# darioShar/DLPM

Measured on AMD Instinct MI355X. Metric: samples/sec at T=1000 (CIFAR-10 32x32, alpha=1.7), higher is better.
Workload: dtype f32 (1x1 / stride-2 convolutions: fp32 operands split exactly into 3 bf16 planes, bf16 MFMA products, fp32 accumulate)

## Files before the change

dlpm_amd/_lib.py:

```python
import ctypes as C
import os

_HERE = os.path.dirname(os.path.abspath(__file__))
LIB_PATH = os.environ.get('DLPM_LIB') or os.path.join(_HERE, 'lib', 'libdlpm_amd.so')

vp, i32, i64, u32, u64, f32, f64 = C.c_void_p, C.c_int32, C.c_int64, C.c_uint32, C.c_uint64, C.c_float, C.c_double

ABI_VERSION = 6
UPD_DLIM, UPD_CLIP, UPD_ADVANCE, SMP_NO_FUSED_MLP, UPD_ELEMENTWISE, SMP_LIM = 1, 2, 4, 8, 16, 32
MEAN_TYPES = {'EPSILON': 0, 'START_X': 1, 'Z': 2, 'PREVIOUS_X': 3}
PRED_TO_XSTART, PRED_CLIP, PRED_TO_EPS, PRED_ELEMENTWISE = 1, 2, 4, 16
LOSS_RESCALE_T, LOSS_ELEMENTWISE = 1, 16
AT_T_Q_SAMPLE, AT_T_PREDICT_EPS, AT_T_PREDICT_XSTART = 0, 1, 2
CONV_AUTO, CONV_F4, CONV_F2, CONV_IGEMM = 0, 1, 2, 3
GEMM_AUTO, GEMM_F32, GEMM_BF16X3 = 0, 1, 2


class MT19937(C.Structure):
    _fields_ = [('key', u32 * 624), ('pos', i32), ('has_cached', i32), ('cached', f64)]


class UpdateArgs(C.Structure):
    _fields_ = [('x_dev', vp), ('eps_dev', vp), ('z_dev', vp), ('t_dev', vp), ('g_dev', vp), ('bg_dev', vp),
                ('bs_dev', vp), ('c_eps_dev', vp), ('c_noise_dev', vp), ('A_dev', vp), ('B', i64), ('D', i64),
# ... 37 lines not shown
                ('conv1_w', vp), ('conv1_b', vp), ('ss', vp), ('ss_stride', i64), ('gn2_w', vp), ('gn2_b', vp), ('conv2_w', vp),
                ('conv2_b', vp), ('skip_w', vp), ('skip_b', vp), ('out', vp), ('stats_out', vp)]


class AttnBlockArgs(C.Structure):
    _fields_ = [('x', vp), ('C', i32), ('heads', i32), ('B', i32), ('H', i32), ('W', i32), ('gn_w', vp), ('gn_b', vp),
                ('qkv_w', vp), ('qkv_b', vp), ('proj_w', vp), ('proj_b', vp), ('out', vp), ('stats_out', vp)]


class SamplerConfig(C.Structure):
    _fields_ = [('unet', vp), ('mlp', vp), ('B', i64), ('C', i32), ('H', i32), ('W', i32), ('T', i32), ('alpha', f64),
                ('clamp_a', f64), ('clamp_eps', f64), ('flags', i32), ('dlim_eta', f32), ('seed', u64),
                ('sample_offset', i64), ('use_graph', i32), ('g', vp), ('bg', vp), ('s', vp), ('bs', vp),
                ('lim_ts', vp), ('lim_tmp', vp), ('lim_cx', vp), ('lim_cs', vp), ('lim_cn', vp), ('in_scale', vp),
                ('mean_type', i32)]


SIGNATURES = {
    'dlpm_last_error': (C.c_char_p, []),
    'dlpm_abi_version': (C.c_int, []),
    'dlpm_prof_enable': (C.c_int, [C.c_int]),
    'dlpm_prof_report': (C.c_int, [C.c_char_p, i64]),
    'dlpm_schedule_f32': (C.c_int, [C.c_int, f64, vp, vp, vp, vp]),
    'dlpm_schedule_exploding_f32': (C.c_int, [C.c_int, f64, vp, vp, vp, vp]),
    'dlpm_mt19937_seed': (C.c_int, [C.POINTER(MT19937), u32]),
    'dlpm_skewed_levy_host_f32': (C.c_int, [C.POINTER(MT19937), f64, i64, f64, vp]),
    'dlpm_randn_host_f32': (C.c_int, [C.POINTER(MT19937), i64, vp]),
    'dlpm_skewed_levy_philox_f32': (C.c_int, [vp, C.c_int, i64, f64, f64, u64, i64, vp]),
    'dlpm_skewed_levy_elem_philox_f32': (C.c_int, [vp, C.c_int, i64, i64, f64, f64, u64, i64, vp]),
    'dlpm_init_state_elem_philox_f32': (C.c_int, [vp, i64, i64, f64, f64, f32, u64, i64, vp]),
    'dlpm_init_state_philox_f32': (C.c_int, [vp, i64, i64, f64, f64, f32, u64, i64, vp]),
    'dlpm_coeff_tables_f32': (C.c_int, [vp, vp, vp, vp, C.c_int, i64, vp, vp, vp, vp]),
    'dlpm_update_f32': (C.c_int, [C.POINTER(UpdateArgs), vp]),
    'dlpm_predict_f32': (C.c_int, [C.POINTER(PredictArgs), vp]),
    'dlpm_fill_scaled_t_f32': (C.c_int, [vp, vp, i32, i64, vp]),
    'dlpm_postprocess_f32': (C.c_int, [vp, vp, i64, f32, C.c_int, vp]),
    'dlpm_scale_by_table_f32': (C.c_int, [vp, vp, i64, vp, vp, vp]),
    'dlpm_lim_tables_f32': (C.c_int, [f64, i32, i32, vp, vp, vp, vp, vp]),
    'dlpm_lim_update_f32': (C.c_int, [C.POINTER(LimUpdateArgs), vp]),
    'dlpm_fill_table_t_f32': (C.c_int, [vp, vp, vp, i32, i64, vp]),
    'dlpm_loss_elements_f32': (C.c_int, [C.POINTER(LossArgs), vp]),
    'dlpm_loss_terms_f32': (C.c_int, [vp, vp, vp, i64, i32, i64, i32, i64, i64, vp]),
    'dlpm_loss_reduce_f32': (C.c_int, [vp, i64, i32, i32, i32, vp, vp, vp, vp]),
    'dlpm_at_t_f32': (C.c_int, [i32, vp, vp, vp, vp, vp, vp, i64, i64, i32, vp]),
    'dlpm_mmd_workspace_bytes': (i64, [i64, i64, i64]),
    'dlpm_mmd_f32': (C.c_int, [vp, i64, vp, i64, i64, f64, i32, f64, vp, i64, vp, vp]),
    'dlpm_images_to_rgb8': (C.c_int, [vp, vp, i64, i32, i32, i32, vp]),
    'dlpm_png_bound': (i64, [i32, i32]),
    'dlpm_png_encode_rgb8': (C.c_int, [vp, i32, i32, i32, vp, i64, C.POINTER(i64)]),
    'dlpm_png_write_rgb8': (C.c_int, [vp, i64, i32, i32, C.c_char_p, i64, i32, i32]),
    'dlpm_unet_create': (C.c_int, [C.POINTER(UNetConfig), C.POINTER(vp)]),
    'dlpm_unet_create_conditional': (C.c_int, [C.POINTER(UNetConfig), i32, C.POINTER(vp)]),
    'dlpm_unet_num_classes': (i32, [vp]),
    'dlpm_unet_set_param': (C.c_int, [vp, C.c_char_p, vp, i64]),
    'dlpm_unet_num_params': (C.c_int, [vp]),
    'dlpm_unet_param_key': (C.c_char_p, [vp, C.c_int, C.POINTER(i64)]),
    'dlpm_unet_finalize': (C.c_int, [vp]),
    'dlpm_unet_workspace_bytes': (i64, [vp, i64]),
    'dlpm_unet_forward': (C.c_int, [vp, vp, vp, vp, i64, vp, i64, vp]),
    'dlpm_unet_forward_uniform_t': (C.c_int, [vp, vp, vp, vp, i64, vp, i64, vp]),
    'dlpm_unet_forward_labels': (C.c_int, [vp, vp, vp, vp, vp, i64, vp, i64, vp]),
    'dlpm_unet_forward_uniform_t_labels': (C.c_int, [vp, vp, vp, vp, vp, i64, vp, i64, vp]),
    'dlpm_unet_forward_update': (C.c_int, [vp, vp, vp, C.POINTER(UpdateArgs), vp, i64, vp, i64, vp]),
    'dlpm_unet_time_embedding_width': (i64, [vp]),
    'dlpm_unet_time_embeddings_scratch_bytes': (i64, [vp, i64]),
    'dlpm_unet_time_embeddings': (C.c_int, [vp, vp, i64, vp, vp, i64, vp]),
    'dlpm_unet_bind_time_table': (C.c_int, [vp, vp, vp]),
    'dlpm_unet_keep_features': (C.c_int, [vp, C.c_int]),
    'dlpm_unet_num_features': (C.c_int, [vp]),
    'dlpm_unet_feature_shape': (C.c_int, [vp, C.c_int, C.POINTER(i32), C.POINTER(i32), C.POINTER(i32)]),
    'dlpm_unet_get_feature': (C.c_int, [vp, C.c_int, vp, i64, vp]),
    'dlpm_unet_flops_per_sample': (i64, [vp]),
    'dlpm_unet_set_conv_policy': (C.c_int, [vp, i32, i64]),
    'dlpm_unet_set_gemm_policy': (C.c_int, [vp, i32]),
    'dlpm_unet_plan_version': (i64, [vp]),
    'dlpm_unet_destroy': (None, [vp]),
    'dlpm_mlp_create': (C.c_int, [i32, i32, i32, i32, C.POINTER(vp)]),
    'dlpm_mlp_set_param': (C.c_int, [vp, C.c_char_p, vp, i64]),
    'dlpm_mlp_finalize': (C.c_int, [vp]),
    'dlpm_mlp_forward': (C.c_int, [vp, vp, vp, vp, i64, vp]),
    'dlpm_mlp_sample_steps_f32': (C.c_int, [vp, vp, vp, vp, vp, i32, i64, i32, i32, u64, i64, vp, vp]),
    'dlpm_mlp_destroy': (None, [vp]),
    'dlpm_conv2d_f32': (C.c_int, [C.POINTER(ConvArgs), vp, vp]),
    'dlpm_groupnorm_coeffs_f32': (C.c_int, [vp, vp, i32, i32, i32, i32, i32, vp, vp, vp, i64, i64, vp, vp, vp]),
    'dlpm_attention_f32': (C.c_int, [vp, vp, i32, i32, i32, i32, vp]),
    'dlpm_attention_general_f32': (C.c_int, [vp, vp, i32, i32, i32, i32, vp]),
    'dlpm_resblock_small_f32': (C.c_int, [C.POINTER(ResBlockArgs), vp, i64, vp]),
    'dlpm_resblock_img_f32': (C.c_int, [C.POINTER(ResBlockArgs), vp, i64, vp]),
    'dlpm_resblock_img_scratch_floats': (i64, [i64, i32]),
    'dlpm_attnblock_small_f32': (C.c_int, [C.POINTER(AttnBlockArgs), vp, i64, vp]),
    'dlpm_timestep_embedding_f32': (C.c_int, [vp, vp, i64, i32, vp]),
    'dlpm_nchw_to_nhwc_f32': (C.c_int, [vp, vp, i32, i32, i32, i32, vp]),
    'dlpm_nhwc_to_nchw_f32': (C.c_int, [vp, vp, i32, i32, i32, i32, vp]),
    'dlpm_sampler_create': (C.c_int, [C.POINTER(SamplerConfig), C.POINTER(vp)]),
    'dlpm_sampler_reseed': (C.c_int, [vp, u64, i64]),
    'dlpm_sampler_begin': (C.c_int, [vp, vp]),
    'dlpm_sampler_begin_injected': (C.c_int, [vp, vp, vp, vp]),
    'dlpm_sampler_set_state': (C.c_int, [vp, vp, i32, vp]),
    'dlpm_sampler_step_injected': (C.c_int, [vp, vp, vp]),
    'dlpm_sampler_steps': (C.c_int, [vp, i32, vp]),
    'dlpm_sampler_set_history': (C.c_int, [vp, vp, vp]),
    'dlpm_sampler_set_labels': (C.c_int, [vp, vp, vp]),
    'dlpm_sampler_copy_state': (C.c_int, [vp, vp, vp]),
    'dlpm_sampler_state': (vp, [vp]),
    'dlpm_sampler_t': (i32, [vp]),
    'dlpm_sampler_table': (vp, [vp, C.c_int]),
    'dlpm_sampler_destroy': (None, [vp]),
}

_lib = None


class DlpmError(RuntimeError):
    pass


def lib():
    global _lib
    if _lib is None:
        if not os.path.exists(LIB_PATH):
            raise DlpmError('libdlpm_amd.so is missing at %s -- run `python -m dlpm_amd.build` '
                            '(or __graft_entry__.build()); there is no CPU fallback' % LIB_PATH)
        handle = C.CDLL(LIB_PATH)
        for name, (res, args) in SIGNATURES.items():
            fn = getattr(handle, name)
            fn.restype = res
            fn.argtypes = args
        got = handle.dlpm_abi_version()
        if got != ABI_VERSION:
            raise DlpmError('libdlpm_amd.so has ABI version %d, the Python mirror expects %d -- rebuild with '
                            '`python -m dlpm_amd.build`' % (got, ABI_VERSION))
        _lib = handle
    return _lib


def check(rc):
    if rc != 0:
        msg = lib().dlpm_last_error().decode('utf-8', 'replace')
        if rc == -1:
            raise ValueError(msg)
        raise DlpmError('[dlpm status %d] %s' % (rc, msg))


def stream_ptr():
    import torch
    return torch.cuda.current_stream().cuda_stream


def ptr(t):
    if t is None:
        return None
    import torch
    assert t.is_contiguous(), 'non-contiguous tensor crossing the C ABI'
    assert t.dtype in (torch.float32, torch.int32), t.dtype
    return t.data_ptr()
```

dlpm_amd/csrc/conv.h:

```cpp
#pragma once
#include "common.h"

namespace dlpm {

struct ConvLaunch {
    const float *src0 = nullptr, *src1 = nullptr;
    int C0 = 0, C1 = 0;
    int B = 0, Hin = 0, Win = 0, Hout = 0, Wout = 0;
    int ks = 1, stride = 1, ups = 0;
    const float *w = nullptr;
    const float *w_frag = nullptr;
    const float *w_wino = nullptr;
    const float *w_wino4 = nullptr;
    const float *w_wino4_n64 = nullptr, *w_wino4_n32 = nullptr;
    const void *w_split = nullptr;
    const float *w_small = nullptr;
    const float *w_taps = nullptr;
    const float *w_hfused = nullptr;
    const float *bias = nullptr;
    const float *coefA = nullptr, *coefB = nullptr;
    int act_silu = 0;
    const float *res0 = nullptr, *res1 = nullptr;
    int R0 = 0;
    float *out = nullptr;
    int Cout = 0;
    int in_nchw = 0, out_nchw = 0;
    int gen = 0;
    int64_t dispatch_B = 0;
    int gemm = 0;
    int ksplit = 0;
    float2 *stats_out = nullptr;
#ifdef DLPM_PHASE_TIMING
    unsigned long long *phase = nullptr;
#endif
};

bool igemm_supported(const ConvLaunch &c);
int launch_conv_igemm(const ConvLaunch &c, hipStream_t st);
int launch_conv_direct(const ConvLaunch &c, hipStream_t st);
int launch_conv_stem(const ConvLaunch &c, hipStream_t st);
struct HeadUpdate {
    float *x = nullptr;
    const float *z = nullptr;
    const int32_t *t = nullptr;
    const float *g = nullptr, *c_eps = nullptr, *c_noise = nullptr;
    const uint64_t *key = nullptr;
    uint64_t seed = 0;
    int64_t sample_offset = 0;
    float *const *hist_pp = nullptr;
    float *eps_out = nullptr;
    int32_t T = 0;
    int64_t B = 0;
};
bool head_conv_ok(const ConvLaunch &c);
int launch_conv_head(const ConvLaunch &c, const HeadUpdate *hu, hipStream_t st);
int relayout_weight_head(const float *oihw_dev, float *dst_dev, int Cout, int Cin, hipStream_t st);
bool head_gemm_ok(const ConvLaunch &c);
int head_taps_rows(int Cout);
int64_t head_gemm_scratch_floats(const ConvLaunch &c);
int launch_conv_head_gemm(const ConvLaunch &c, const HeadUpdate *hu, float *P, hipStream_t st);
int relayout_weight_head_taps(const float *oihw_dev, float *dst_dev, int Cout, int Cin, hipStream_t st);
bool head_fused_ok(const ConvLaunch &c);
int64_t head_fused_weight_floats(int Cin);
int relayout_weight_head_fused(const float *oihw_dev, float *dst_dev, int Cout, int Cin, hipStream_t st);
int launch_conv_head_fused(const ConvLaunch &c, const HeadUpdate *hu, hipStream_t st);
bool wino_geometry(const ConvLaunch &c, int *bh, int *bw, int *nimg);
int wino_tiles(const ConvLaunch &c);
int launch_conv_wino(const ConvLaunch &c, hipStream_t st);
int64_t wino_weight_floats(int Cout, int Cin);
int relayout_weight_wino(const float *oihw_dev, float *dst_dev, int Cout, int Cin, hipStream_t st);
bool wino4_enabled();
bool wino4_geometry(const ConvLaunch &c, int *bh, int *bw, int *nimg);
bool wino4_preferred(const ConvLaunch &c, int *bh, int *bw, int *nimg);
int launch_conv_wino4(const ConvLaunch &c, hipStream_t st);
int64_t wino4_weight_floats(int Cout, int Cin);
int relayout_weight_wino4(const float *oihw_dev, float *dst_dev, int Cout, int Cin, hipStream_t st, int nq = 0);
struct ResImgLaunch {
    const float *x0 = nullptr, *x1 = nullptr;
    int C0 = 0, C1 = 0, B = 0;
    int H = 32;
    const float2 *st0 = nullptr, *st1 = nullptr;
    int nt0 = 1, nt1 = 1;
    const float *coefA1 = nullptr, *coefB1 = nullptr;
    const float *gn1_w = nullptr, *gn1_b = nullptr, *gn2_w = nullptr, *gn2_b = nullptr;
    const float *w1 = nullptr, *b1 = nullptr;
    const float *w2 = nullptr, *b2 = nullptr;
    const float *emb = nullptr;
    int64_t emb_stride = 0;
    int emb_off = 0;
    const float *res = nullptr;
    float *hbuf = nullptr;
    float *out = nullptr;
    float2 *stats_out = nullptr;
#ifdef DLPM_PHASE_TIMING
    unsigned long long *phase = nullptr;
#endif
};
bool res_img_ok(const ResImgLaunch &r);
int launch_resblock_img(const ResImgLaunch &r, hipStream_t st);

bool conv_split_ok(const ConvLaunch &c);
int launch_conv_split(const ConvLaunch &c, hipStream_t st);
int64_t split_weight_floats(int Cout, int Cin, int taps);
int relayout_weight_split(const float *oihw_dev, void *dst_dev, int Cout, int Cin, int taps, hipStream_t st);
int conv_stats_pixels(const ConvLaunch &c);
int conv_ksplit_for(const ConvLaunch &c);
int wino4_launch_nq(const ConvLaunch &c);
int64_t wino_grid_at(const ConvLaunch &c, int64_t B);
int launch_splitk_reduce(const float *part, int S, int64_t npix, int Cout, const float *bias, const float *res0, const float *res1, int R0,
                         float *out, hipStream_t st);
inline int launch_conv_fallback(const ConvLaunch &L, hipStream_t st) {
    if (L.in_nchw && !L.out_nchw && L.ks == 3 && L.stride == 1 && !L.ups && L.C1 == 0 && L.Cout % 4 == 0 && !L.coefA &&
        !L.act_silu && !L.res0 && L.bias)
        return launch_conv_stem(L, st);
    return launch_conv_direct(L, st);
}

int relayout_weight(const float *oihw_dev, float *dst_dev, int Cout, int Cin, int ks, bool for_igemm, hipStream_t st);
int64_t frag_weight_floats(int Cout, int Cin);
int relayout_weight_frag(const float *oihw_dev, float *dst_dev, int Cout, int Cin, hipStream_t st);

int launch_gn_coeffs(const float *src0, const float *src1, int C0, int C1, int B, int HW, int groups,
                     const float *gamma, const float *beta, const float *ss, int64_t ss_stride, int64_t ss_offset,
                     float *coefA, float *coefB, hipStream_t st);
int launch_gn_coeffs_from_stats(const float2 *st0, const float2 *st1, int C0, int C1, int B, int nt0, int nt1, int HW, int groups,
                                const float *gamma, const float *beta, const float *ss, int64_t ss_stride,
                                int64_t ss_offset, float *coefA, float *coefB, hipStream_t st);
int launch_attention(const float *qkv, float *out, int B, int T, int C, int heads, hipStream_t st);
int launch_attention_general(const float *qkv, float *out, int B, int T, int C, int heads, hipStream_t st);

struct ResSmallLaunch {
    const float *x0 = nullptr, *x1 = nullptr;
    int C0 = 0, C1 = 0, B = 0, H = 0, W = 0;
    const float *gn1_w = nullptr, *gn1_b = nullptr, *gn2_w = nullptr, *gn2_b = nullptr;
    const float *w1f = nullptr, *b1 = nullptr;
    const float *w2f = nullptr, *b2 = nullptr;
    const float *wsf = nullptr, *bs = nullptr;
    const float *emb = nullptr;
    int64_t emb_stride = 0;
    int emb_off = 0;
    float *out = nullptr;
    float2 *stats_out = nullptr;
};
struct AttnSmallLaunch {
    const float *x = nullptr;
    int C = 0, heads = 0, B = 0, H = 0, W = 0;
    const float *gn_w = nullptr, *gn_b = nullptr;
    const float *wqkv = nullptr, *bqkv = nullptr;
    const float *wproj = nullptr, *bproj = nullptr;
    float *out = nullptr;
    float2 *stats_out = nullptr;
#ifdef DLPM_PHASE_TIMING
    unsigned long long *phase = nullptr;
#endif
};
bool attn_small_ok(const AttnSmallLaunch &a);
int launch_attnblock_small(const AttnSmallLaunch &a, hipStream_t st);
bool attn16_ok(const AttnSmallLaunch &a);
int launch_attnblock16(const AttnSmallLaunch &a, hipStream_t st);
// ... 18 lines not shown
```

dlpm_amd/csrc/conv_igemm.hip:

```cpp
#include <cstdlib>

#include <algorithm>

#include "conv.h"
#include "igemm_epilogue.h"

namespace dlpm {
namespace {

constexpr int KC = 32;
constexpr int LDS_LD = 36;

template <int BN, int WAVES_M, int WAVES_N, int RM, int RN>
__device__ __forceinline__ void epilogue_rows(const ConvLaunch &p, floatx16 (&acc)[RM][RN], float *lds, int64_t m0, int n0,
                                              int64_t M, int tid, int wm, int wn, int l31, int kh) {
    constexpr int LD = BN + 4, PR = RM * 32, C4 = BN / 4, RG = 256 / C4;
    const int R1 = p.Cout - p.R0;
    const bool do_stats = p.stats_out != nullptr;
    float4 K = make_float4(0.f, 0.f, 0.f, 0.f), s1 = K, s2 = K;
    int cnt = 0;
    for (int ph = 0; ph < WAVES_M; ph++) {
        if (wm == ph) {
#pragma unroll
            for (int i = 0; i < RM; i++)
// ... 913 lines not shown
    return *nimg * (*th + 2) * (W + 2) * 8 <= HALO_NIT * 256;
}

template <int BN, int WAVES_M, int WAVES_N, int RM, int RN, int RING, bool UPS>
static int launch_halo_ws_r(const ConvLaunch &c, int th, int nimg, int64_t grid, hipStream_t st) {
    const int hp = nimg * ((UPS ? th / 2 : th) + 2) * ((UPS ? c.Wout / 2 : c.Wout) + 2);
    size_t shmem = (size_t)((hp + 3) & ~3) * LDS_LD * sizeof(float) + (size_t)nimg * 64 * sizeof(float);
    const size_t epi = (size_t)(RM * 32) * (BN + 4) * sizeof(float);
    const size_t stats = (size_t)(256 / (BN / 4)) * BN * 2 * sizeof(float);
    if (shmem < epi) shmem = epi;
    if (shmem < stats) shmem = stats;
    {
        int r = ensure_dynamic_lds(reinterpret_cast<const void *>(&k_conv3x3_halo_ws<BN, WAVES_M, WAVES_N, RM, RN, RING, UPS>), 64 * 1024);
        if (r != DLPM_OK) return r;
    }
    k_conv3x3_halo_ws<BN, WAVES_M, WAVES_N, RM, RN, RING, UPS><<<(unsigned)grid, 256, shmem, st>>>(c, th, nimg);
    return DLPM_OK;
}

template <int BN, int WAVES_M, int WAVES_N, int RM, int RN>
static int launch_halo_ws(const ConvLaunch &c, int th, int nimg, int64_t grid, hipStream_t st) {
    if (c.ups) return launch_halo_ws_r<BN, WAVES_M, WAVES_N, RM, RN, 2, true>(c, th, nimg, grid, st);
    return launch_halo_ws_r<BN, WAVES_M, WAVES_N, RM, RN, 2, false>(c, th, nimg, grid, st);
}

template <int BN, int WAVES_M, int WAVES_N, int RM, int RN>
static int launch_halo(const ConvLaunch &c, int th, int nimg, int64_t grid, hipStream_t st) {
    const int hp = nimg * (th + 2) * (c.Wout + 2);
    const size_t shmem = (size_t)(((hp + 3) & ~3) + 2 * BN) * LDS_LD * sizeof(float) + (size_t)nimg * 64 * sizeof(float);
    {
        int r = ensure_dynamic_lds(reinterpret_cast<const void *>(&k_conv3x3_halo<BN, WAVES_M, WAVES_N, RM, RN>), 100 * 1024);
        if (r != DLPM_OK) return r;
    }
    k_conv3x3_halo<BN, WAVES_M, WAVES_N, RM, RN><<<(unsigned)grid, 256, shmem, st>>>(c, th, nimg);
    return DLPM_OK;
}

static bool stem_stats_ok(const ConvLaunch &c) {
    const int Cq = c.Cout / 4;
    return c.in_nchw && !c.out_nchw && c.ks == 3 && c.stride == 1 && !c.ups && c.C1 == 0 && (c.C0 == 3 || c.C0 == 1) && c.Cout % 4 == 0 &&
           Cq >= 1 && Cq <= 256 && (Cq & (Cq - 1)) == 0 && ((int64_t)c.Hout * c.Wout) % 1024 == 0;
}

int launch_conv_stem(const ConvLaunch &c, hipStream_t st) {
    const int64_t total = (int64_t)c.B * c.Hout * c.Wout * (c.Cout / 4);
    ProfScope ps("conv_stem", 2.0 * total * 4 * c.C0 * 9, 4.0 * ((double)c.B * c.Hin * c.Win * c.C0 + total * 4.0), st);
    const int Cq = c.Cout / 4;
    const bool regw = Cq >= 1 && Cq <= 256 && (Cq & (Cq - 1)) == 0;
    const int64_t Mpix = (int64_t)c.B * c.Hout * c.Wout;
    const int ppb = 1024;
    if (c.stats_out && !stem_stats_ok(c)) {
        set_error("launch_conv_stem: statistics requested for a shape that cannot emit them");
        return DLPM_ERR_UNSUPPORTED;
    }
    static int nolds = -1;
    if (nolds < 0) { const char *e = getenv("DLPM_NO_STEM_LDS"); nolds = (e && e[0] == '1') ? 1 : 0; }
    const int W = c.Wout;
    const bool lds_ok = !nolds && regw && c.Hin == c.Hout && c.Win == c.Wout && (W & (W - 1)) == 0 && W >= 4 && W <= 64 && ppb % W == 0 &&
                        ((int64_t)c.Hout * W) % ppb == 0 && c.bias;
    if (lds_ok && (c.C0 == 3 || c.C0 == 1)) {
        const size_t shmem = std::max((size_t)(ppb / W + 2) * (W + 2) * sizeof(float4), (size_t)(256 / Cq) * c.Cout * sizeof(float2));
        if (c.C0 == 3) k_conv_stem_lds<3><<<(unsigned)(Mpix / ppb), 256, shmem, st>>>(c, ppb);
        else k_conv_stem_lds<1><<<(unsigned)(Mpix / ppb), 256, shmem, st>>>(c, ppb);
        DLPM_LAUNCH_CHECK();
        return DLPM_OK;
    }
    if (c.C0 == 3 && regw) k_conv_stem_regw<3><<<(unsigned)ceil_div(Mpix, ppb), 256, 0, st>>>(c, ppb);
    else if (c.C0 == 1 && regw) k_conv_stem_regw<1><<<(unsigned)ceil_div(Mpix, ppb), 256, 0, st>>>(c, ppb);
    else if (c.C0 == 3) k_conv_stem<3><<<(unsigned)ceil_div(total, 256), 256, 0, st>>>(c);
    else if (c.C0 == 1) k_conv_stem<1><<<(unsigned)ceil_div(total, 256), 256, 0, st>>>(c);
    else return launch_conv_direct(c, st);
    DLPM_LAUNCH_CHECK();
    return DLPM_OK;
}

int conv_stats_pixels(const ConvLaunch &c) {
    int a, b, n;
    if (conv_ksplit_for(c) > 1) return 0;
    if (c.in_nchw) return stem_stats_ok(c) ? 1024 : 0;
    if (conv_split_ok(c)) {
        const int64_t hw = (int64_t)c.Hout * c.Wout;
        return (c.R0 & 3) ? 0 : hw % BM == 0 ? BM : hw == 64 ? 64 : 0;
    }
    if (wino4_preferred(c, &a, &b, &n)) return n == 1 ? 256 : (n == 4 && a * b == 4) ? 64 : 0;
    if (wino_geometry(c, &a, &b, &n)) return n == 1 ? 4 * wino_tiles(c) : 0;
    if (c.out_nchw || (c.Cout & 3) || (c.R0 & 3)) return 0;
    return ((int64_t)c.Hout * c.Wout) % BM == 0 ? BM : 0;
}

int launch_conv_igemm(const ConvLaunch &c, hipStream_t st) {
    const int64_t M = (int64_t)c.B * c.Hout * c.Wout;
    const int64_t mt = ceil_div(M, BM);
    const double K = (double)(c.C0 + c.C1) * c.ks * c.ks;
    const double bytes = 4.0 * ((double)c.B * c.Hin * c.Win * (c.C0 + c.C1) + K * c.Cout + (double)M * c.Cout * (c.res0 ? 2 : 1));
    char pname[96];
    int th = 0, nimg = 1;
    if (prof_enabled() && prof_detail())
        snprintf(pname, sizeof(pname), "conv%dx%d_igemm:H%d:Cin%d+%d:Cout%d:s%d:u%d:coef%d", c.ks, c.ks, c.Hout, c.C0, c.C1, c.Cout,
                 c.stride, c.ups, c.coefA ? 1 : 0);
    else
        snprintf(pname, sizeof(pname), "%s", c.ks == 3 ? (halo_ok(c, &th, &nimg) ? "conv3x3_halo" : "conv3x3_igemm") : "conv1x1_igemm");
    if (conv_split_ok(c)) {
        if (prof_enabled() && prof_detail())
            snprintf(pname, sizeof(pname), "conv%dx%d_bf16x3:H%d:Cin%d+%d:Cout%d:s%d:coef%d", c.ks, c.ks, c.Hout, c.C0, c.C1, c.Cout, c.stride,
                     c.coefA ? 1 : 0);
        else
            snprintf(pname, sizeof(pname), c.ks == 1 ? "conv1x1_bf16x3" : "conv3x3_bf16x3");
        ProfScope pss(pname, 2.0 * M * c.Cout * K, bytes + 2.0 * K * c.Cout, st);
#ifdef DLPM_PHASE_TIMING
        const_cast<ConvLaunch &>(c).phase = phase_buffer();
#endif
        return launch_conv_split(c, st);
    }
    {
        int wb, ww, wi;
        if (wino4_preferred(c, &wb, &ww, &wi)) {
            if (prof_enabled() && prof_detail())
                snprintf(pname, sizeof(pname), "conv3x3_wino4:H%d:Cin%d+%d:Cout%d:u%d:coef%d", c.Hout, c.C0, c.C1, c.Cout, c.ups, c.coefA ? 1 : 0);
            else
                snprintf(pname, sizeof(pname), "conv3x3_wino4");
            ProfScope psw(pname, 2.0 * M * c.Cout * K, bytes, st);
            return launch_conv_wino4(c, st);
        }
        if (wino_geometry(c, &wb, &ww, &wi)) {
            if (prof_enabled() && prof_detail())
                snprintf(pname, sizeof(pname), "conv3x3_wino:H%d:Cin%d+%d:Cout%d:u%d:coef%d", c.Hout, c.C0, c.C1, c.Cout, c.ups, c.coefA ? 1 : 0);
            else
                snprintf(pname, sizeof(pname), "conv3x3_wino");
            ProfScope psw(pname, 2.0 * M * c.Cout * K, bytes, st);
            return launch_conv_wino(c, st);
        }
    }
    ProfScope ps(pname, 2.0 * M * c.Cout * K, bytes, st);
#ifdef DLPM_PHASE_TIMING
    const_cast<ConvLaunch &>(c).phase = phase_buffer();
#endif
    if (halo_ok(c, &th, &nimg)) {
        int r;
        if (c.w_frag && !ws_disabled() && (c.C0 + c.C1) % KC == 0) {
            if (c.Cout > 64) r = launch_halo_ws<128, 2, 2, 2, 2>(c, th, nimg, mt * ceil_div(c.Cout, 128), st);
            else if (c.Cout > 32) r = launch_halo_ws<64, 2, 2, 2, 1>(c, th, nimg, mt * ceil_div(c.Cout, 64), st);
            else r = launch_halo_ws<32, 4, 1, 1, 1>(c, th, nimg, mt * ceil_div(c.Cout, 32), st);
            if (r != DLPM_OK) return r;
            DLPM_LAUNCH_CHECK();
            return DLPM_OK;
        }
        if (c.Cout > 64) r = launch_halo<128, 2, 2, 2, 2>(c, th, nimg, mt * ceil_div(c.Cout, 128), st);
        else if (c.Cout > 32) r = launch_halo<64, 2, 2, 2, 1>(c, th, nimg, mt * ceil_div(c.Cout, 64), st);
        else r = launch_halo<32, 4, 1, 1, 1>(c, th, nimg, mt * ceil_div(c.Cout, 32), st);
        if (r != DLPM_OK) return r;
        DLPM_LAUNCH_CHECK();
        return DLPM_OK;
    }
    static int nofast = -1;
    if (nofast < 0) { const char *e = getenv("DLPM_NO_FAST_IGEMM"); nofast = (e && e[0] == '1') ? 1 : 0; }
    const int bn = c.Cout > 64 ? 128 : c.Cout > 32 ? 64 : 32;
    const bool full = !nofast && M % BM == 0 && c.Cout % bn == 0 && !c.out_nchw && (c.R0 & 3) == 0;
    const bool g1 = full && c.ks == 1 && c.stride == 1 && !c.ups && !c.in_nchw && c.C0 % KC == 0 && (c.C0 + c.C1) % KC == 0;
    const int mode = g1 ? 2 : full ? 1 : 0;
    const unsigned grid = (unsigned)(mt * ceil_div(c.Cout, bn));
#define DLPM_IGEMM_LAUNCH(BN_, WM_, WN_, RM_, RN_)                                                   \
    do {                                                                                             \
        if (mode == 2) k_conv_igemm<BN_, WM_, WN_, RM_, RN_, 2><<<grid, 256, 0, st>>>(c);            \
        else if (mode == 1) k_conv_igemm<BN_, WM_, WN_, RM_, RN_, 1><<<grid, 256, 0, st>>>(c);       \
        else k_conv_igemm<BN_, WM_, WN_, RM_, RN_, 0><<<grid, 256, 0, st>>>(c);                      \
    } while (0)
    if (bn == 128) DLPM_IGEMM_LAUNCH(128, 2, 2, 2, 2);
    else if (bn == 64) DLPM_IGEMM_LAUNCH(64, 2, 2, 2, 1);
    else DLPM_IGEMM_LAUNCH(32, 4, 1, 1, 1);
#undef DLPM_IGEMM_LAUNCH
    DLPM_LAUNCH_CHECK();
    return DLPM_OK;
}

int64_t frag_weight_floats(int Cout, int Cin) {
    return ((int64_t)((Cout + 31) / 32) * (Cin / 32) * 9 * 4 + 2) * 256;
}

int relayout_weight_frag(const float *oihw_dev, float *dst_dev, int Cout, int Cin, hipStream_t st) {
    const int64_t n = (int64_t)((Cout + 31) / 32) * (Cin / 32) * 9 * 4 * 256;
    DLPM_HIP(hipMemsetAsync(dst_dev + n, 0, 2 * 256 * sizeof(float), st));
    k_relayout_weight_frag<<<(unsigned)ceil_div(n, 256), 256, 0, st>>>(oihw_dev, dst_dev, Cout, Cin);
    DLPM_LAUNCH_CHECK();
    return DLPM_OK;
}

int relayout_weight(const float *oihw_dev, float *dst_dev, int Cout, int Cin, int ks, bool for_igemm, hipStream_t st) {
    const int64_t n = (int64_t)Cout * Cin * ks * ks;
    k_relayout_weight<<<(unsigned)ceil_div(n, 256), 256, 0, st>>>(oihw_dev, dst_dev, Cout, Cin, ks, for_igemm ? 1 : 0);
    DLPM_LAUNCH_CHECK();
    return DLPM_OK;
}

}
```

dlpm_amd/csrc/conv_wino4.hip:

```cpp
#include <cstdlib>
#include <type_traits>

#include "conv.h"
#include "gn_stats.h"

namespace dlpm {
namespace {

typedef float floatx4 __attribute__((ext_vector_type(4)));

constexpr int F4_TILES = 16;
constexpr int F4_NQ = 128;
constexpr int F4_KC = 8;
constexpr int F4_RAWPIX = 576;
constexpr int F4_PRLD = F4_KC + 4;
constexpr int F4_NT = 512;
constexpr int F4_QNIT = (F4_RAWPIX * 2 + F4_NT - 1) / F4_NT;
constexpr int F4_RAWBUF = F4_RAWPIX * F4_PRLD + 16;
constexpr int F4_RAWPIX_N = 400;
constexpr int F4_RAWBUF_N = F4_RAWPIX_N * F4_PRLD + 16;
constexpr int f4_nq_of(int cout) { return cout % 128 == 0 ? 128 : cout % 64 == 0 ? 64 : 32; }
constexpr int F4_CFS = 16 * 2 * F4_KC;
constexpr int F4_VBUF = 36 * F4_TILES * F4_KC;
#ifndef F4_RING_DEPTH
// ... 100 lines not shown
        f4_v_row_out(Ta, vb + 0 * 3 * vpp, vpp);
    } else {
#pragma unroll
        for (int c = 0; c < 6; c++) f4_bt_mid<3>(d, c, Ta[c], Tb[c]);
        f4_v_row_out(Ta, vb + 3 * 3 * vpp, vpp);
        f4_v_row_out(Tb, vb + 4 * 3 * vpp, vpp);
#pragma unroll
        for (int c = 0; c < 6; c++) Tb[c] = f4_bt_outer<5>(d, c);
        f4_v_row_out(Tb, vb + 5 * 3 * vpp, vpp);
    }
}

__device__ __forceinline__ void f4_at(float m0, float m1, float m2, float m3, float m4, float m5, float &y0, float &y1, float &y2, float &y3) {
    const float s12 = m1 + m2, d12 = m1 - m2, s34 = m3 + m4, d34 = m3 - m4;
    y0 = m0 + s12 + s34;
    y1 = fmaf(PB, d34, PA * d12);
    y2 = fmaf(PB2, s34, PA2 * s12);
    y3 = fmaf(PB3, d34, PA3 * d12) + m5;
}
__device__ __forceinline__ void f4_out_tile(const floatx4 (&acc)[36], int r, float (&Yt)[16]) {
    float Z[4][6];
#pragma unroll
    for (int b = 0; b < 6; b++)
        f4_at(acc[0 * 6 + b][r], acc[1 * 6 + b][r], acc[2 * 6 + b][r], acc[3 * 6 + b][r], acc[4 * 6 + b][r], acc[5 * 6 + b][r], Z[0][b], Z[1][b],
              Z[2][b], Z[3][b]);
#pragma unroll
    for (int i = 0; i < 4; i++) f4_at(Z[i][0], Z[i][1], Z[i][2], Z[i][3], Z[i][4], Z[i][5], Yt[i * 4 + 0], Yt[i * 4 + 1], Yt[i * 4 + 2], Yt[i * 4 + 3]);
}

template <int N>
__device__ __forceinline__ void f4_stats_lane(float K, float s1, float s2, float &mean, float &M2) {
    mean = K + s1 * (1.f / N);
    M2 = fmaxf(s2 - s1 * s1 * (1.f / N), 0.f);
}
template <int N>
__device__ __forceinline__ void f4_stats_merge(float K, float s1, float s2, int lane, float &mean, float &M2) {
    f4_stats_lane<N>(K, s1, s2, mean, M2);
    float na = (float)N;
#pragma unroll
    for (int sft = 16; sft <= 32; sft <<= 1) {
        const float om = __shfl_xor(mean, sft), oM2 = __shfl_xor(M2, sft);
        const float lo_m = (lane & sft) ? om : mean, hi_m = (lane & sft) ? mean : om;
        const float lo_M = (lane & sft) ? oM2 : M2, hi_M = (lane & sft) ? M2 : oM2;
        const float dd = hi_m - lo_m;
        mean = lo_m + dd * 0.5f;
        M2 = lo_M + hi_M + dd * dd * (na * 0.5f);
        na *= 2.f;
    }
}

__device__ __forceinline__ void f4_mfma4(float4 aa, float4 b, floatx4 &acc0, floatx4 &acc1) {
    acc0 = __builtin_amdgcn_mfma_f32_16x16x4f32(aa.x, b.x, acc0, 0, 0, 0);
    acc1 = __builtin_amdgcn_mfma_f32_16x16x4f32(aa.z, b.z, acc1, 0, 0, 0);
    acc0 = __builtin_amdgcn_mfma_f32_16x16x4f32(aa.y, b.y, acc0, 0, 0, 0);
    acc1 = __builtin_amdgcn_mfma_f32_16x16x4f32(aa.w, b.w, acc1, 0, 0, 0);
}
__device__ __forceinline__ void f4_mfma_pair(int pp, const float *asrc, int vpp, const float4 *wp, int lane, float4 (&aq)[2], float4 (&bq)[F4_RING],
                                             floatx4 (&acc)[36]) {
    constexpr int AHEAD = F4_RING - 1;
    if (pp == 0) aq[0] = *reinterpret_cast<const float4 *>(asrc);
    if (pp + AHEAD < 18) bq[(pp + AHEAD) % F4_RING] = wp[(pp + AHEAD) * 64 + lane];
    if (pp + 1 < 18) aq[(pp + 1) & 1] = *reinterpret_cast<const float4 *>(asrc + (pp + 1) * vpp);
    f4_mfma4(aq[pp & 1], bq[pp % F4_RING], acc[2 * pp], acc[2 * pp + 1]);
}

__device__ __forceinline__ float4 f4_affine4(float4 x, float4 ca, float4 cb) {
    return make_float4(fmaf(x.x, ca.x, cb.x), fmaf(x.y, ca.y, cb.y), fmaf(x.z, ca.z, cb.z), fmaf(x.w, ca.w, cb.w));
}
__device__ __forceinline__ float4 f4_silu4(float4 x) { return make_float4(silu_f(x.x), silu_f(x.y), silu_f(x.z), silu_f(x.w)); }
__device__ __forceinline__ float4 f4_affine_silu4(float4 x, float4 ca, float4 cb) { return f4_silu4(f4_affine4(x, ca, cb)); }
template <int W, int PRLD>
__device__ __forceinline__ int f4_item_pack(int pix, int ch) {
    constexpr int RW = W + 2;
    const int ry = pix / RW, rx = pix - ry * RW;
    const int iy = ry - 1, ix = rx - 1;
    const bool pad = iy < 0 || iy >= W || ix < 0 || ix >= W;
    const int lo = pix * PRLD + ch + 4 * (ry >> 2);
    return pix >= RW * RW ? (1 << 25) : (lo | (pad ? (1 << 24) : ((iy * W + ix) << 14)));
}
__device__ __forceinline__ int f4_item_lds(int iv) { return iv & 16383; }
__device__ __forceinline__ int f4_item_src(int iv) { return (iv >> 14) & 1023; }
__device__ __forceinline__ bool f4_item_pad(int iv) { return iv & (1 << 24); }
__device__ __forceinline__ bool f4_item_none(int iv) { return iv & (1 << 25); }

template <bool UPS, int QN = F4_QNIT, int NW = 8>
__global__ void __launch_bounds__((NW + (NW == 8 ? 0 : NW == 4 ? 3 : 2)) * 64, NW == 2 ? 2 : 1) k_conv3x3_wino4(ConvLaunch p_in, int bh_in, int bw_in, int nimg_in) {
    constexpr bool HELP = NW != 8;
    constexpr int NH = NW == 8 ? 0 : NW == 4 ? 3 : 2;
    constexpr int F4_NT = (NW + NH) * 64, F4_NQ = NW * 16;
    constexpr int F4_RAWBUF = NW == 8 ? dlpm::F4_RAWBUF : F4_RAWBUF_N;
    ConvLaunch p = p_in;
    const int bh = bh_in, bw = bw_in, nimg = nimg_in;
    extern __shared__ __attribute__((aligned(16))) float wsm[];
    float *V = wsm;
    float *raw = wsm + 2 * F4_VBUF;
    float *Cf = raw + 2 * F4_RAWBUF;

    DLPM_PHASE_DECL;
#ifdef DLPM_PHASE_TIMING
    const long long _c0 = clock64(), _r0 = wall_clock64();
#endif
#ifdef DLPM_PHASE_TIMING
    long long _wait = 0;
#endif
    const int tid = threadIdx.x, lane = tid & 63, wave = tid >> 6;
    const bool mfma_wave = !HELP || wave < NW;
    const int li = lane & 15, lk = lane >> 4;
    const int W = p.Wout, H = p.Hout, TW = W >> 2, TH = H >> 2;
    const int Ws = UPS ? (W >> 1) : W, Hs = UPS ? (H >> 1) : H;
    const int Cin = p.C0 + p.C1;
    int nch = Cin / F4_KC, kb = 0;
    unsigned bid = blockIdx.x, nblk = gridDim.x;
    if constexpr (HELP) {
        if (p.ksplit > 1) {
            nblk = gridDim.x / p.ksplit;
            const int ks = (int)(blockIdx.x / nblk);
            bid = blockIdx.x - (unsigned)ks * nblk;
            nch /= p.ksplit;
            kb = ks * nch;
            p.out += (int64_t)ks * p.B * H * W * p.Cout;
        }
    }
    const int ntn = p.Cout / F4_NQ;
    const int nmb = nblk / ntn;
    const int mb = bid % nmb, n0 = (bid / nmb) * F4_NQ;
    int img0, ty0, tx0, blk_in_img = 0;
    if (nimg == 1) {
        const int bpr = TW / bw, bpi = (TH / bh) * bpr;
        img0 = mb / bpi;
        blk_in_img = mb - img0 * bpi;
        ty0 = (blk_in_img / bpr) * bh;
        tx0 = (blk_in_img % bpr) * bw;
    } else {
        img0 = mb * nimg;
        ty0 = tx0 = 0;
    }
    const int RH = UPS ? 2 * bh + 2 : 4 * bh + 2, RW = UPS ? 2 * bw + 2 : 4 * bw + 2;
    const int oy = UPS ? 2 * ty0 - 1 : 4 * ty0 - 1, ox = UPS ? 2 * tx0 - 1 : 4 * tx0 - 1;
    const int rpi = RH * RW, npix = nimg * rpi;

    const int squad = tid & 1;
    auto pix_of = [&](int it) { return it == 1 ? (F4_NT / 2) + ((F4_NT - 1 - tid) >> 1) : it * (F4_NT / 2) + (tid >> 1); };
    const bool skewed = !UPS && nimg == 1 && bh <= 4;
    int off[QN], lo[QN];
#pragma unroll
    for (int it = 0; it < QN; it++) {
        const int pix = pix_of(it);
        const int img = min(pix / rpi, nimg - 1), r = pix - img * rpi;
        const int ry = r / RW, rx = r - ry * RW;
        const int iy = oy + ry, ix = ox + rx;
        const bool pad = iy < 0 || iy >= Hs || ix < 0 || ix >= Ws || (img0 + img) >= p.B;
        off[it] = pix >= npix ? -2 : (pad ? -1 : (((img0 + img) * Hs + iy) * Ws + ix));
        lo[it] = (pix * F4_PRLD + squad * 4 + (skewed ? 4 * (ry >> 2) : 0)) | ((img * 2 * F4_KC + squad * 4) << 16);
    }
    const bool has_coef = p.coefA != nullptr;
    const int cf_img = tid >> 2, cf_isb = (tid >> 1) & 1;
    const bool cf_mine = has_coef && tid < nimg * 4;
    const float *cf_base = has_coef ? ((cf_isb ? p.coefB : p.coefA) + (int64_t)min(img0 + cf_img, p.B - 1) * Cin + kb * F4_KC + squad * 4) : nullptr;
    float4 xr[QN], cfr = make_float4(0.f, 0.f, 0.f, 0.f);
    auto load_raw_into = [&](float4 (&dst)[QN], int chunk) {
        const int c = (kb + chunk) * F4_KC + squad * 4;
        const bool first = c < p.C0;
        const float *sb = first ? p.src0 + c : p.src1 + (c - p.C0);
        const int ld = first ? p.C0 : p.C1;
#pragma unroll
        for (int it = 0; it < QN; it++) dst[it] = *reinterpret_cast<const float4 *>(sb + (int64_t)max(off[it], 0) * ld);
// ... 134 lines not shown
    if (p.phase && lane == 0) atomicAdd(p.phase + 16 + wave, (unsigned long long)_wait);
#endif

    const int64_t pix0 = ((int64_t)img0 * H + 4 * ty0) * W + 4 * tx0;
    const int ch = n0 + 16 * wave + li;
    const float bias_v = p.bias ? p.bias[ch] : 0.f;
    const bool has_res = p.res0 != nullptr;
    const bool res_first = __builtin_amdgcn_readfirstlane(n0 + 16 * wave) < p.R0;
    const float *res_u = has_res ? (res_first ? p.res0 : p.res1 - p.R0) : nullptr;
    const int res_ld = res_first ? p.R0 : p.Cout - p.R0;
    const int lbw = 31 - __builtin_clz(bw), lbhw = 31 - __builtin_clz(bh * bw);
    float *__restrict__ out_blk = p.out + pix0 * p.Cout;
    const float *__restrict__ res_blk = has_res ? res_u + pix0 * res_ld : nullptr;
    const bool img_stats = p.stats_out != nullptr && nimg == 4 && bh * bw == 4;
    const bool do_stats = (p.stats_out != nullptr && nimg == 1) || img_stats;
    float K = 0.f, s1 = 0.f, s2 = 0.f;
    float rs_all[HELP ? 4 : 1][16] = {};
#pragma unroll
    for (int r = 0; r < 4; r++) {
        const int tile = 4 * lk + r;
        const int timg = tile >> lbhw, ty = (tile & (bh * bw - 1)) >> lbw, tx = tile & (bw - 1);
        const int tpix = (timg * H + 4 * ty) * W + 4 * tx;
        const bool ok = img0 + timg < p.B;
        float rs[16];
        const uint32_t bo_o = (uint32_t)(tpix * p.Cout + ch) * 4u, bo_r = (uint32_t)(tpix * res_ld + ch) * 4u;
        if (HELP) {
            if (r == 0 && has_res) {
#pragma unroll
                for (int rr = 0; rr < 4; rr++) {
                    const int t2 = 4 * lk + rr;
                    const int tp2 = ((t2 >> lbhw) * H + 4 * ((t2 & (bh * bw - 1)) >> lbw)) * W + 4 * (t2 & (bw - 1));
                    const uint32_t b2 = (uint32_t)(tp2 * res_ld + ch) * 4u;
                    const bool ok2 = img0 + (t2 >> lbhw) < p.B;
#pragma unroll
                    for (int k = 0; k < 16; k++)
                        rs_all[rr][k] = ok2 ? *reinterpret_cast<const float *>(reinterpret_cast<const char *>(res_blk + ((k >> 2) * W + (k & 3)) * res_ld) + b2) : 0.f;
                }
            }
#pragma unroll
            for (int k = 0; k < 16; k++) rs[k] = rs_all[r][k];
        } else if (has_res && ok) {
#pragma unroll
            for (int i = 0; i < 4; i++)
#pragma unroll
                for (int j = 0; j < 4; j++)
                    rs[i * 4 + j] = *reinterpret_cast<const float *>(reinterpret_cast<const char *>(res_blk + (i * W + j) * res_ld) + bo_r);
        }
        float Yt[16];
        f4_out_tile(acc, r, Yt);
        if (!ok) continue;
#pragma unroll
        for (int i = 0; i < 4; i++) {
            const float *y = Yt + 4 * i;
#pragma unroll
            for (int j = 0; j < 4; j++) {
                float v = y[j] + bias_v;
                if (has_res) v += rs[i * 4 + j];
                if (do_stats) {
                    if (r == 0 && i == 0 && j == 0) K = v;
                    const float dd = v - K;
                    s1 += dd;
                    s2 = fmaf(dd, dd, s2);
                }
                *reinterpret_cast<float *>(reinterpret_cast<char *>(out_blk + (i * W + j) * p.Cout) + bo_o) = v;
            }
        }
    }
    if (img_stats) {
        if (img0 + lk < p.B) {
            float mean, M2;
            f4_stats_lane<64>(K, s1, s2, mean, M2);
            p.stats_out[(int64_t)(img0 + lk) * p.Cout + ch] = make_float2(mean, M2);
        }
    } else if (do_stats) {
        float mean, M2;
        f4_stats_merge<64>(K, s1, s2, lane, mean, M2);
        if (lk == 0) p.stats_out[((int64_t)img0 * ((H * W) / 256) + blk_in_img) * p.Cout + ch] = make_float2(mean, M2);
    }
    DLPM_PHASE(p, 10);
    DLPM_PHASE_FLUSH(p, 8);
#ifdef DLPM_PHASE_DEFER
    if (p.phase && lane == 0) atomicAdd(p.phase + 16 + wave, (unsigned long long)_wait);
#endif
#ifdef DLPM_PHASE_TIMING
    if (p.phase && tid == 0) {
        atomicAdd(p.phase + 11, 1ull);
        atomicAdd(p.phase + 12, (unsigned long long)(clock64() - _c0));
        atomicAdd(p.phase + 13, (unsigned long long)(wall_clock64() - _r0));
    }
#endif
}

constexpr int FI_TILES = 64, FI_RW = 34, FI_NPIX = FI_RW * FI_RW, FI_NT = 512;
constexpr int FI_QN = (FI_NPIX * 2 + FI_NT - 1) / FI_NT;
constexpr int FI_RAWBUF = FI_NPIX * F4_PRLD + 48;
constexpr int FI_VPP = 4 * FI_TILES * 4;
constexpr int FI_VBUF = 18 * FI_VPP;

#define F4_LDS_BARRIER()                                                  \
    do {                                                                  \
        __builtin_amdgcn_fence(__ATOMIC_RELEASE, "workgroup", "local");   \
        __builtin_amdgcn_s_barrier();                                     \
        __builtin_amdgcn_fence(__ATOMIC_ACQUIRE, "workgroup", "local");   \
    } while (0)

__global__ void __launch_bounds__(FI_NT, 1) k_conv3x3_wino4_img(ConvLaunch p) {
    extern __shared__ __attribute__((aligned(16))) float wsm[];
    float *V = wsm;
    float *raw = V + FI_VBUF;
    float *Cf = raw + FI_RAWBUF;
    DLPM_PHASE_DECL;
#ifdef DLPM_PHASE_TIMING
    const long long _c0 = clock64(), _r0 = wall_clock64();
#endif
    constexpr int H = 32, W = 32;
    const int tid = threadIdx.x, lane = tid & 63, wave = __builtin_amdgcn_readfirstlane(tid >> 6);
    const int li = lane & 15, lk = lane >> 4;
    const int mb = wave >> 1, nw = wave & 1;
    const int img = blockIdx.x;
    const int Cin = p.C0 + p.C1, nch = Cin / F4_KC, last = nch - 1;
    const bool has_coef = p.coefA != nullptr;

    const int squad = tid & 1;
    int itm[FI_QN];
#pragma unroll
    for (int it = 0; it < FI_QN; it++) itm[it] = f4_item_pack<W, F4_PRLD>(it * (FI_NT / 2) + (tid >> 1), squad * 4);
    float4 xr[FI_QN];
    auto load_raw = [&](int chunk) {
        const int c = chunk * F4_KC + squad * 4;
        const bool first = c < p.C0;
        const int ld = first ? p.C0 : p.C1;
        const float *sb = (first ? p.src0 + c : p.src1 + (c - p.C0)) + (int64_t)img * (H * W) * ld;
#pragma unroll
        for (int it = 0; it < FI_QN; it++) xr[it] = *reinterpret_cast<const float4 *>(sb + f4_item_src(itm[it]) * ld);
    };
    auto store_raw = [&](int chunk) {
        const int c = chunk * F4_KC + squad * 4;
        float4 ca = make_float4(1.f, 1.f, 1.f, 1.f), cb = make_float4(0.f, 0.f, 0.f, 0.f);
        if (has_coef) {
            ca = *reinterpret_cast<const float4 *>(Cf + c);
            cb = *reinterpret_cast<const float4 *>(Cf + Cin + c);
        }
#pragma unroll
        for (int it = 0; it < FI_QN; it++) {
            int iv = itm[it];
            asm volatile("" : "+v"(iv));
            if (f4_item_none(iv)) continue;
            float4 x = xr[it];
            if (has_coef) x = f4_affine4(x, ca, cb);
            if (p.act_silu) x = f4_silu4(x);
            if (f4_item_pad(iv)) x = make_float4(0.f, 0.f, 0.f, 0.f);
            *reinterpret_cast<float4 *>(raw + f4_item_lds(iv)) = x;
        }
    };

    int rbase, vofs;
    {
        const int tg = wave & 3, tile = lane & 15, pair = lane >> 4;
        const int ty = 4 * (tg >> 1) + (tile >> 2), tx = 4 * (tg & 1) + (tile & 3);
        rbase = (4 * ty * FI_RW + 4 * tx) * F4_PRLD + pair * 2 + 4 * ty;
        vofs = (pair * FI_TILES + 16 * tg + tile) * 4;
    }
    const int th = wave >> 2;
    auto transform = [&]() { f4_transform_half(th, F4Patch<false, F4_PRLD>{raw + rbase, FI_RW, true}, V + vofs, FI_VPP); };

    const float4 *__restrict__ wp = reinterpret_cast<const float4 *>(p.w_wino4) + (int64_t)nw * nch * 18 * 64;
// ... 485 lines not shown
    auto epilogue = [&](auto ra_c) __attribute__((always_inline)) {
        constexpr int RA = decltype(ra_c)::value;
        exchange(ra_c);
        int chv = ch, lkv = lk;
        asm volatile("" : "+v"(chv), "+v"(lkv));
        const float bias_v = p.b2[chv];
        const int64_t pix0 = (int64_t)img * H * W;
        float *__restrict__ out_blk = p.out + pix0 * CO;
        const float *__restrict__ res_blk = p.res + pix0 * CO;
        const bool do_stats = p.stats_out != nullptr;
        float K = 0.f, s1 = 0.f, s2 = 0.f;
        auto one = [&](auto r_c, int rr) __attribute__((always_inline)) {
            const int tile = 4 * lkv + RA + rr;
            const int tpix = (4 * (tile >> 2)) * W + 4 * (tile & 3);
            float rs[16];
#pragma unroll
            for (int k = 0; k < 16; k++) rs[k] = res_blk[(tpix + (k >> 2) * W + (k & 3)) * CO + chv];
            float Yt[16];
            f4_out_tile(acc, decltype(r_c)::value, Yt);
#pragma unroll
            for (int k = 0; k < 16; k++) {
                const float v = (Yt[k] + bias_v) + rs[k];
                if (rr == 0 && k == 0) K = v;
                const float dd = v - K;
                s1 += dd;
                s2 = fmaf(dd, dd, s2);
                out_blk[(tpix + (k >> 2) * W + (k & 3)) * CO + chv] = v;
            }
        };
        one(std::integral_constant<int, RA>(), 0);
        one(std::integral_constant<int, RA + 1>(), 1);
        if (do_stats) {
            float mean, M2;
            f4_stats_merge<32>(K, s1, s2, lane, mean, M2);
            if (lkv == 0) part[kh * CO + chv] = make_float2(mean, M2);
            F4_LDS_BARRIER();
            if (kh == 0 && lkv == 0) {
                const float2 a = part[chv], b = part[CO + chv];
                const float dd = b.x - a.x;
                p.stats_out[(int64_t)img * CO + chv] = make_float2(a.x + dd * 0.5f, a.y + b.y + dd * dd * 64.f);
            }
        }
    };
    if (kh == 0) epilogue(std::integral_constant<int, 0>());
    else epilogue(std::integral_constant<int, 2>());
    DLPM_PHASE(p, 10);
    DLPM_PHASE_FLUSH(p, 8);
#ifdef DLPM_PHASE_TIMING
    if (p.phase && tid == 0) atomicAdd(p.phase + 11, 1ull);
#endif
}

__global__ void k_relayout_weight_wino4(const float *oihw, float *dst, int Cout, int Cin, int nw) {
    const int nch = Cin / F4_KC;
    const int64_t total = (int64_t)Cout * Cin * 36;
    const int64_t i = (int64_t)blockIdx.x * blockDim.x + threadIdx.x;
    if (i >= total) return;
    const int e = (int)(i & 3);
    const int lane = (int)((i >> 2) & 63);
    int64_t r = i >> 8;
    const int pp = (int)(r % 18); r /= 18;
    const int chunk = (int)(r % nch); r /= nch;
    const int wave = (int)(r % nw);
    const int nt = (int)(r / nw);
    const int lk = lane >> 4, li = lane & 15;
    const int pos = 2 * pp + (e >> 1);
    const int cin = chunk * F4_KC + 2 * lk + (e & 1);
    const int cout = nt * (16 * nw) + wave * 16 + li;
    const float *g = oihw + ((int64_t)cout * Cin + cin) * 9;
    const double a = F4_PA, b = F4_PB, a2 = a * a, b2 = b * b;
    const double n0 = a2 * b2, na = 2. * a2 * (a2 - b2), nb = 2. * b2 * (b2 - a2);
    const double G[6][3] = {{1. / n0, 0., 0.},         {1. / na, a / na, a2 / na}, {1. / na, -a / na, a2 / na},
                            {1. / nb, b / nb, b2 / nb}, {1. / nb, -b / nb, b2 / nb}, {0., 0., 1.}};
    const int ra = pos / 6, rb = pos % 6;
    double u = 0.;
    for (int ii = 0; ii < 3; ii++) {
        double row = 0.;
        for (int jj = 0; jj < 3; jj++) row += (double)g[ii * 3 + jj] * G[rb][jj];
        u += G[ra][ii] * row;
    }
    dst[i] = (float)u;
}

int f4_mode() {
    static int v = -1;
    if (v < 0) { const char *e = getenv("DLPM_WINO_F4"); v = e ? atoi(e) : 1; }
    return v;
}

}

bool wino4_enabled() { return f4_mode() != 0; }

static bool narrow_enabled() {
    static int v = -1;
    if (v < 0) { const char *e = getenv("DLPM_WINO4_NARROW"); v = e ? atoi(e) : 1; }
    return v != 0;
}

static bool wino4_geometry_nq(const ConvLaunch &c, int nq, int *bh, int *bw, int *nimg) {
    if (nq != F4_NQ && !narrow_enabled()) return false;
    if (!c.w_wino4 || c.ks != 3 || c.stride != 1 || c.in_nchw || c.out_nchw) return false;
    if ((c.Hout & 3) || (c.Wout & 3) || c.Cout % 32 != 0 || (c.C0 + c.C1) % F4_KC != 0 || c.C0 % F4_KC != 0) return false;
    const int rawpix = nq == F4_NQ ? F4_RAWPIX : F4_RAWPIX_N;
    if ((c.R0 & 15) != 0) return false;
    const int TH = c.Hout / 4, TW = c.Wout / 4;
    int h, w, n;
    if (TH * TW >= F4_TILES) {
        w = TW < 4 ? TW : 4;
        if (F4_TILES % w != 0) return false;
        h = F4_TILES / w;
        if (TW % w != 0 || TH % h != 0) return false;
        n = 1;
    } else {
        if (F4_TILES % (TH * TW) != 0) return false;
        h = TH; w = TW; n = F4_TILES / (TH * TW);
    }
    const int RH = c.ups ? 2 * h + 2 : 4 * h + 2, RW = c.ups ? 2 * w + 2 : 4 * w + 2;
    if (n * RH * RW > rawpix) return false;
    *bh = h; *bw = w; *nimg = n;
    return true;
}

static int wino4_nq_for(const ConvLaunch &c) {
    const int base = f4_nq_of(c.Cout);
    if (base != F4_NQ || c.dispatch_B <= 0 || (!c.w_wino4_n64 && !c.w_wino4_n32)) return base;
    static int floor_nq = -1;
    if (floor_nq < 0) { const char *e = getenv("DLPM_WINO4_NQ"); floor_nq = e ? atoi(e) : 32; }
    int best = F4_NQ;
    for (int nq = F4_NQ; nq >= 32 && nq >= floor_nq; nq >>= 1) {
        if (nq == 64 && !c.w_wino4_n64) continue;
        if (nq == 32 && !c.w_wino4_n32) continue;
        int h, w, n;
        if (!wino4_geometry_nq(c, nq, &h, &w, &n)) continue;
        best = nq;
        const int64_t tiles = c.dispatch_B * (c.Hout / 4) * (c.Wout / 4);
        const int64_t mblocks = n == 1 ? tiles / F4_TILES : ceil_div(c.dispatch_B, (int64_t)n);
        if (mblocks * (c.Cout / nq) >= 256) break;
    }
    return best;
}

bool wino4_geometry(const ConvLaunch &c, int *bh, int *bw, int *nimg) { return wino4_geometry_nq(c, wino4_nq_for(c), bh, bw, nimg); }
int wino4_launch_nq(const ConvLaunch &c) { return wino4_nq_for(c); }

bool wino4_preferred(const ConvLaunch &c, int *bh, int *bw, int *nimg) {
    if (c.gen == DLPM_CONV_F2 || c.gen == DLPM_CONV_IGEMM) return false;
    if (!wino4_geometry(c, bh, bw, nimg)) return false;
    if (!c.w_wino || c.gen == DLPM_CONV_F4) return true;
    if (*nimg > 4) return false;
    if (c.dispatch_B <= 0) return true;
    const int64_t tiles = c.dispatch_B * (c.Hout / 4) * (c.Wout / 4);
    const int64_t mblocks = *nimg == 1 ? tiles / F4_TILES : ceil_div(c.dispatch_B, (int64_t)*nimg);
    return mblocks * (c.Cout / wino4_nq_for(c)) >= 256;
}

static bool wino4_whole_image(const ConvLaunch &c) {
    static int v = -1;
    if (v < 0) { const char *e = getenv("DLPM_WINO4_IMG"); v = e ? atoi(e) : 1; }
    return v != 0 && c.Cout == 32 && !c.ups && c.Hout == 32 && c.Wout == 32 && (c.C0 + c.C1) <= 1024;
}

static int launch_conv_wino4_nq(const ConvLaunch &c, int nq, int bh, int bw, int nimg, hipStream_t st);

int launch_conv_wino4(const ConvLaunch &c, hipStream_t st) {
    int bh, bw, nimg;
// ... 31 lines not shown
        KFn fn = nq == 64 ? (c.ups ? &k_conv3x3_wino4<true, 2, 4> : &k_conv3x3_wino4<false, 2, 4>)
                          : (c.ups ? &k_conv3x3_wino4<true, 4, 2> : &k_conv3x3_wino4<false, 4, 2>);
        const int r = ensure_dynamic_lds(reinterpret_cast<const void *>(fn), 160 * 1024);
        if (r != DLPM_OK) return r;
        const size_t lds = (size_t)(2 * F4_VBUF + 2 * F4_RAWBUF_N + 2 * F4_CFS) * sizeof(float);
        const int ks = c.ksplit > 1 ? c.ksplit : 1;
        if (ks > 1 && (c.bias || c.res0 || c.stats_out || ((c.C0 + c.C1) / F4_KC) % ks != 0)) {
            set_error("launch_conv_wino4: a split-K launch carries no bias / residual / statistics and divides its chunks evenly");
            return DLPM_ERR_ARG;
        }
        fn<<<(unsigned)(mblocks * (c.Cout / nq) * ks), (nq == 64 ? 7 : 4) * 64, lds, st>>>(c, bh, bw, nimg);
        DLPM_LAUNCH_CHECK();
        return DLPM_OK;
    }
    if (c.ksplit > 1) {
        set_error("launch_conv_wino4: split-K is a narrow-shape launch");
        return DLPM_ERR_ARG;
    }
    const int RHp = c.ups ? 2 * bh + 2 : 4 * bh + 2, RWp = c.ups ? 2 * bw + 2 : 4 * bw + 2;
    const bool small = nimg * RHp * RWp <= F4_NT;
    KFn fn = c.ups ? (small ? &k_conv3x3_wino4<true, 2> : &k_conv3x3_wino4<true>) : (small ? &k_conv3x3_wino4<false, 2> : &k_conv3x3_wino4<false>);
    const int r = ensure_dynamic_lds(reinterpret_cast<const void *>(fn), 160 * 1024);
    if (r != DLPM_OK) return r;
    const size_t lds = (size_t)(2 * F4_VBUF + 2 * F4_RAWBUF + 2 * F4_CFS) * sizeof(float);
    fn<<<(unsigned)(mblocks * (c.Cout / F4_NQ)), F4_NT, lds, st>>>(c, bh, bw, nimg);
    DLPM_LAUNCH_CHECK();
    return DLPM_OK;
}

bool res_img_ok(const ResImgLaunch &r) {
    static int v = -1;
    if (v < 0) { const char *e = getenv("DLPM_RES_IMG"); v = e ? atoi(e) : 1; }
    const int Cin = r.C0 + r.C1;
    const bool common = v != 0 && wino4_enabled() && r.w1 && r.w2 && r.res && Cin <= 128 && Cin >= 32 &&
                        (r.st0 ? (r.C1 == 0 || r.st1 != nullptr) : (r.coefA1 && r.coefB1));
    if (r.H == 16) {
        static int v16 = -1;
        if (v16 < 0) { const char *e = getenv("DLPM_RES_IMG16"); v16 = e ? atoi(e) : 1; }
        return common && v16 != 0 && Cin % F6_KC == 0 && r.C0 % F6_KC == 0;
    }
    return common && r.H == 32 && r.hbuf && Cin % F4_KC == 0 && r.C0 % F4_KC == 0;
}

int launch_resblock_img(const ResImgLaunch &r, hipStream_t st) {
    if (!res_img_ok(r)) {
        set_error("launch_resblock_img: unsupported block");
        return DLPM_ERR_UNSUPPORTED;
    }
    const int Cin = r.C0 + r.C1;
#ifdef DLPM_PHASE_TIMING
    const_cast<ResImgLaunch &>(r).phase = phase_buffer();
#endif
    if (r.H == 16) {
        const double M16 = (double)r.B * 256;
        ProfScope ps16("resblock_img:H16", 2.0 * M16 * 64 * 9.0 * (Cin + 64), 4.0 * (M16 * (Cin + 64 + 64) + 64 * 9.0 * (Cin + 64)), st);
        const int e16 = ensure_dynamic_lds(reinterpret_cast<const void *>(&k_resblock_wino4_img16), 160 * 1024);
        if (e16 != DLPM_OK) return e16;
        const size_t lds16 = (size_t)(F6_VBUF + F6_RAWBUF + F6_HBUF + 256 + 512 + 256 + F6_QN * FI_NT) * sizeof(float);
        k_resblock_wino4_img16<<<(unsigned)r.B, FI_NT, lds16, st>>>(r);
        DLPM_LAUNCH_CHECK();
        return DLPM_OK;
    }
    const double M = (double)r.B * 1024;
    ProfScope ps("resblock_img:H32", 2.0 * M * 32 * 9.0 * (Cin + 32), 4.0 * (M * (Cin + 32 + 32) + 32 * 9.0 * (Cin + 32)), st);
    const int e = ensure_dynamic_lds(reinterpret_cast<const void *>(&k_resblock_wino4_img), 160 * 1024);
    if (e != DLPM_OK) return e;
    const size_t lds = (size_t)(FI_VBUF + FI_RAWBUF + 256 + 512 + 256 + FI_QN * FI_NT) * sizeof(float);
    k_resblock_wino4_img<<<(unsigned)r.B, FI_NT, lds, st>>>(r);
    DLPM_LAUNCH_CHECK();
    return DLPM_OK;
}

int64_t wino4_weight_floats(int Cout, int Cin) { return (int64_t)Cout * Cin * 36 + F4_PAD * 256; }

int relayout_weight_wino4(const float *oihw_dev, float *dst_dev, int Cout, int Cin, hipStream_t st, int nq_in) {
    const int64_t n = (int64_t)Cout * Cin * 36;
    DLPM_HIP(hipMemsetAsync(dst_dev + n, 0, (size_t)F4_PAD * 256 * sizeof(float), st));
    const int nq = nq_in > 0 ? nq_in : f4_nq_of(Cout);
    k_relayout_weight_wino4<<<(unsigned)ceil_div(n, 256), 256, 0, st>>>(oihw_dev, dst_dev, Cout, Cin, nq / 16);
    DLPM_LAUNCH_CHECK();
    return DLPM_OK;
}

}
```

dlpm_amd/csrc/unet.hip:

```cpp
#include <cmath>
#include <cstdlib>
#include <map>
#include <string>
#include <utility>
#include <vector>

#include "conv.h"

using namespace dlpm;

namespace {

struct Param {
    std::string key;
    int64_t numel = 0;
    float *dev = nullptr;
    bool set = false;
};

enum LayerKind { L_STEM, L_RES, L_ATTN, L_DOWN, L_UP };

struct ConvW {
    int p_w = -1, p_b = -1;
    int cout = 0, cin = 0, ks = 1;
    bool use_igemm = false;
    float *w_dev = nullptr;
    float *w_frag = nullptr;
    float *w_wino = nullptr;
    float *w_wino4 = nullptr;
    float *w_wino4_n64 = nullptr, *w_wino4_n32 = nullptr;
    float *w_small = nullptr;
    float *w_taps = nullptr;
    void *w_split = nullptr;
    float *w_rs = nullptr;
    float *w_hfused = nullptr;
    bool owns = false;
};

struct Layer {
    LayerKind kind;
    std::string pre;
    int cin = 0, cout = 0;
    int emb_off = 0;
    ConvW c1, c2, skip;
    bool has_skip = false;
    int p_gn1_w = -1, p_gn1_b = -1, p_gn2_w = -1, p_gn2_b = -1;
    int p_emb_w = -1, p_emb_b = -1;
};

struct Tensor4 {
    float *p = nullptr;
    int C = 0, H = 0, W = 0;
    float2 *stats = nullptr;
    int stats_px = 0;
};

struct Bump {
    char *base = nullptr;
    int64_t cap = 0, off = 0, peak = 0;
    bool dry = false, overflow = false, reuse = true;
    std::vector<std::pair<int64_t, int64_t>> holes;
    std::map<int64_t, int64_t> live;
    char *origin() const { return dry ? reinterpret_cast<char *>(uintptr_t(1) << 20) : base; }
    float *alloc(int64_t nfloats) {
        const int64_t bytes = (nfloats * 4 + 255) / 256 * 256;
        int64_t at = -1;
        if (reuse) {
            size_t best = holes.size();
            for (size_t i = 0; i < holes.size(); i++)
                if (holes[i].second >= bytes && (best == holes.size() || holes[i].second < holes[best].second)) best = i;
            if (best != holes.size()) {
                at = holes[best].first;
                if (holes[best].second == bytes) holes.erase(holes.begin() + best);
                else { holes[best].first += bytes; holes[best].second -= bytes; }
            }
        }
        if (at < 0) {
            at = off;
            off += bytes;
            if (off > peak) peak = off;
            if (!dry && off > cap) overflow = true;
        }
        live[at] = bytes;
        return reinterpret_cast<float *>(origin() + at);
    }
    void release(const void *p) {
        if (!p || !reuse) return;
        const int64_t at = reinterpret_cast<const char *>(p) - origin();
        auto it = live.find(at);
        if (it == live.end()) return;
        int64_t lo = at, n = it->second;
        live.erase(it);
        size_t i = 0;
        while (i < holes.size() && holes[i].first < lo) i++;
        if (i > 0 && holes[i - 1].first + holes[i - 1].second == lo) { lo = holes[i - 1].first; n += holes[i - 1].second; holes.erase(holes.begin() + --i); }
        if (i < holes.size() && lo + n == holes[i].first) { n += holes[i].second; holes.erase(holes.begin() + i); }
        if (lo + n == off) { off = lo; return; }
        holes.insert(holes.begin() + i, std::make_pair(lo, n));
    }
};

void policy_of(const dlpm_unet *u, ConvLaunch &L);

void plan_stats(const dlpm_unet *u, Bump &ws, Tensor4 &t, const ConvW &c, int B, int C0, int stride, int ups, bool stem = false) {
    static int off = -1;
    if (off < 0) { const char *e = getenv("DLPM_NO_GN_FUSION"); off = (e && e[0] == '1') ? 1 : 0; }
    t.stats = nullptr;
    t.stats_px = 0;
    if (off || (!c.use_igemm && !stem)) return;
    ConvLaunch L;
    L.w_wino = c.w_wino; L.w_wino4 = c.w_wino4; L.w_wino4_n64 = c.w_wino4_n64; L.w_wino4_n32 = c.w_wino4_n32; L.w_split = c.w_split; L.ks = c.ks; L.stride = stride; L.ups = ups; L.Hout = t.H; L.Wout = t.W; L.Cout = c.cout;
    L.Hin = ups ? t.H / 2 : t.H * stride; L.Win = ups ? t.W / 2 : t.W * stride;
    L.C0 = C0; L.C1 = c.cin - C0; L.B = B;
    L.in_nchw = stem ? 1 : 0;
    policy_of(u, L);
    const int px = conv_stats_pixels(L);
    if (px <= 0) return;
    t.stats_px = px;
    t.stats = reinterpret_cast<float2 *>(ws.alloc((int64_t)2 * B * (t.H * t.W / px) * t.C));
}

int gn_any(Tensor4 x0, Tensor4 x1, int B, int groups, const float *gamma, const float *beta, const float *ss,
           int64_t ss_stride, int64_t ss_offset, float *cA, float *cB, hipStream_t st) {
    const int HW = x0.H * x0.W;
    if (x0.stats && (x1.C == 0 || x1.stats))
        return launch_gn_coeffs_from_stats(x0.stats, x1.stats, x0.C, x1.C, B, HW / x0.stats_px, x1.C ? HW / x1.stats_px : 1, HW,
                                           groups, gamma, beta, ss, ss_stride, ss_offset, cA, cB, st);
    return launch_gn_coeffs(x0.p, x1.p, x0.C, x1.C, B, HW, groups, gamma, beta, ss, ss_stride, ss_offset, cA, cB, st);
}


void drop(Bump &ws, Tensor4 &t) {
    ws.release(t.p);
    ws.release(t.stats);
    t.p = nullptr;
    t.stats = nullptr;
}

}

struct dlpm_unet {
    dlpm_unet_config cfg;
    std::vector<Param> params;
    std::map<std::string, int> index;
    std::vector<std::vector<Layer>> in_blocks, out_blocks;
    std::vector<Layer> mid;
    std::vector<int> skip_ch;
    ConvW te0, te2, embcat, head;
    int p_head_gn_w = -1, p_head_gn_b = -1;
    float *embcat_w = nullptr, *embcat_b = nullptr;
    int emb_total = 0, ted = 0, final_ch = 0;
    int num_classes = 0;
    int p_label = -1;
    bool finalized = false;
    std::vector<Tensor4> feats;
    int64_t flops = 0;
    bool keep_feats = false;
    int gen = DLPM_CONV_AUTO;
    int64_t dispatch_B = 0;
    int gemm = DLPM_GEMM_AUTO;
    int64_t plan_version = 0;

    int add(const std::string &key, int64_t numel) {
        Param p;
        p.key = key;
        p.numel = numel;
        params.push_back(p);
        index[key] = (int)params.size() - 1;
        return (int)params.size() - 1;
    }
    ConvW conv(const std::string &pre, int cout, int cin, int ks) {
        ConvW c;
        c.cout = cout; c.cin = cin; c.ks = ks;
        c.p_w = add(pre + "weight", (int64_t)cout * cin * ks * ks);
        c.p_b = add(pre + "bias", cout);
        return c;
    }
    Layer res(const std::string &pre, int cin, int cout) {
        Layer L;
        L.kind = L_RES; L.pre = pre; L.cin = cin; L.cout = cout;
        L.p_gn1_w = add(pre + "in_layers.0.weight", cin);
        L.p_gn1_b = add(pre + "in_layers.0.bias", cin);
        L.c1 = conv(pre + "in_layers.2.", cout, cin, 3);
        L.p_emb_w = add(pre + "emb_layers.1.weight", (int64_t)2 * cout * ted);
        L.p_emb_b = add(pre + "emb_layers.1.bias", 2 * cout);
        L.p_gn2_w = add(pre + "out_layers.0.weight", cout);
        L.p_gn2_b = add(pre + "out_layers.0.bias", cout);
        L.c2 = conv(pre + "out_layers.3.", cout, cout, 3);
        L.has_skip = cin != cout;
        if (L.has_skip) L.skip = conv(pre + "skip_connection.", cout, cin, 1);
        L.emb_off = emb_total;
        emb_total += 2 * cout;
        return L;
    }
// ... 9 lines not shown
    bool has_attn(int ds) const {
        for (int i = 0; i < cfg.n_attn; i++)
            if (cfg.attention_resolutions[i] == ds) return true;
        return false;
    }
};

namespace {

void policy_of(const dlpm_unet *u, ConvLaunch &L) {
    L.gen = u->gen;
    L.dispatch_B = u->dispatch_B;
    L.gemm = u->gemm;
}

void build_arch(dlpm_unet *u) {
    const dlpm_unet_config &c = u->cfg;
    const int mc = c.model_channels;
    u->ted = 4 * mc;
    u->te0 = u->conv("time_embed.0.", u->ted, mc, 1);
    u->te2 = u->conv("time_embed.2.", u->ted, u->ted, 1);
    if (u->num_classes > 0) u->p_label = u->add("label_emb.weight", (int64_t)u->num_classes * u->ted);
    {
        Layer L;
        L.kind = L_STEM; L.pre = "input_blocks.0.0."; L.cin = c.in_channels; L.cout = mc;
        L.c1 = u->conv(L.pre, mc, c.in_channels, 3);
        u->in_blocks.push_back({L});
        u->skip_ch.push_back(mc);
    }
    int ch = mc, ds = 1;
    for (int level = 0; level < c.n_mult; level++) {
        const int mult = c.channel_mult[level];
        for (int r = 0; r < c.num_res_blocks; r++) {
            const std::string pre = "input_blocks." + std::to_string(u->in_blocks.size()) + ".";
            std::vector<Layer> seq;
            seq.push_back(u->res(pre + "0.", ch, mult * mc));
            ch = mult * mc;
            if (u->has_attn(ds)) seq.push_back(u->attn(pre + "1.", ch));
            u->in_blocks.push_back(seq);
            u->skip_ch.push_back(ch);
        }
        if (level != c.n_mult - 1) {
            Layer L;
            L.kind = L_DOWN; L.pre = "input_blocks." + std::to_string(u->in_blocks.size()) + ".0.op.";
            L.cin = L.cout = ch;
            L.c1 = u->conv(L.pre, ch, ch, 3);
            u->in_blocks.push_back({L});
            u->skip_ch.push_back(ch);
            ds *= 2;
        }
    }
    u->mid.push_back(u->res("middle_block.0.", ch, ch));
    u->mid.push_back(u->attn("middle_block.1.", ch));
    u->mid.push_back(u->res("middle_block.2.", ch, ch));
    std::vector<int> stack = u->skip_ch;
    for (int level = c.n_mult - 1; level >= 0; level--) {
        const int mult = c.channel_mult[level];
        for (int i = 0; i <= c.num_res_blocks; i++) {
            const std::string pre = "output_blocks." + std::to_string(u->out_blocks.size()) + ".";
            const int ich = stack.back();
            stack.pop_back();
            std::vector<Layer> seq;
            seq.push_back(u->res(pre + "0.", ch + ich, mc * mult));
            ch = mc * mult;
            int k = 1;
            if (u->has_attn(ds)) seq.push_back(u->attn(pre + std::to_string(k++) + ".", ch));
            if (level && i == c.num_res_blocks) {
                Layer L;
                L.kind = L_UP; L.pre = pre + std::to_string(k++) + ".conv.";
                L.cin = L.cout = ch;
                L.c1 = u->conv(L.pre, ch, ch, 3);
                seq.push_back(L);
                ds /= 2;
            }
            u->out_blocks.push_back(seq);
        }
    }
    u->final_ch = ch;
    u->p_head_gn_w = u->add("out.0.weight", ch);
    u->p_head_gn_b = u->add("out.0.bias", ch);
    u->head = u->conv("out.2.", c.out_channels, mc, 3);
}

int prep_conv(dlpm_unet *u, ConvW &c, int C0, int boundary) {
    ConvLaunch probe;
    probe.C0 = C0; probe.C1 = c.cin - C0; probe.Cout = c.cout; probe.ks = c.ks;
    probe.in_nchw = boundary == 1; probe.out_nchw = boundary == 2;
    c.use_igemm = igemm_supported(probe);
    const float *src = u->params[c.p_w].dev;
    if (c.use_igemm && c.ks == 1) {
        c.w_dev = const_cast<float *>(src);
        if (small_weight_ok(c.cout, c.cin, 1) && boundary == 0) {
            DLPM_HIP(hipMalloc(&c.w_rs, (size_t)small_weight_floats(c.cout, c.cin, 1) * sizeof(float)));
            int r = relayout_weight_small(src, c.w_rs, c.cout, c.cin, 1, nullptr);
            if (r != DLPM_OK) return r;
        }
        if (c.cout % 128 == 0 && c.cin % 32 == 0 && boundary == 0) {
            DLPM_HIP(hipMalloc(&c.w_split, (size_t)split_weight_floats(c.cout, c.cin, 1) * sizeof(float)));
            return relayout_weight_split(src, c.w_split, c.cout, c.cin, 1, nullptr);
        }
        return DLPM_OK;
    }
    DLPM_HIP(hipMalloc(&c.w_dev, (size_t)c.cout * c.cin * c.ks * c.ks * sizeof(float)));
    c.owns = true;
    if (c.ks == 3 && c.cout <= 4 && c.cin % 32 == 0) {
        DLPM_HIP(hipMalloc(&c.w_small, (size_t)9 * c.cin * 4 * sizeof(float)));
        int r = relayout_weight_head(src, c.w_small, c.cout, c.cin, nullptr);
        if (r != DLPM_OK) return r;
        if (c.cout <= 3) {
            DLPM_HIP(hipMalloc(&c.w_taps, (size_t)head_taps_rows(c.cout) * c.cin * sizeof(float)));
            r = relayout_weight_head_taps(src, c.w_taps, c.cout, c.cin, nullptr);
            if (r != DLPM_OK) return r;
            if (c.cin <= 128) {
                DLPM_HIP(hipMalloc(&c.w_hfused, (size_t)head_fused_weight_floats(c.cin) * sizeof(float)));
                r = relayout_weight_head_fused(src, c.w_hfused, c.cout, c.cin, nullptr);
                if (r != DLPM_OK) return r;
            }
        }
    }
    if (c.use_igemm && c.ks == 3 && boundary == 4 && c.cout % 128 == 0 && c.cin % 32 == 0) {
        DLPM_HIP(hipMalloc(&c.w_split, (size_t)split_weight_floats(c.cout, c.cin, 9) * sizeof(float)));
        int r = relayout_weight_split(src, c.w_split, c.cout, c.cin, 9, nullptr);
        if (r != DLPM_OK) return r;
    }
    if (c.use_igemm && c.ks == 3 && c.cin % 32 == 0) {
        DLPM_HIP(hipMalloc(&c.w_frag, (size_t)frag_weight_floats(c.cout, c.cin) * sizeof(float)));
        int r = relayout_weight_frag(src, c.w_frag, c.cout, c.cin, nullptr);
        if (r != DLPM_OK) return r;
        if (c.cout % 64 == 0 && c.cin % 16 == 0 && boundary == 0) {
            DLPM_HIP(hipMalloc(&c.w_wino, (size_t)wino_weight_floats(c.cout, c.cin) * sizeof(float)));
            r = relayout_weight_wino(src, c.w_wino, c.cout, c.cin, nullptr);
            if (r != DLPM_OK) return r;
        }
        if (wino4_enabled() && c.cout % 32 == 0 && c.cin % 8 == 0 && boundary == 0) {
            DLPM_HIP(hipMalloc(&c.w_wino4, (size_t)wino4_weight_floats(c.cout, c.cin) * sizeof(float)));
            r = relayout_weight_wino4(src, c.w_wino4, c.cout, c.cin, nullptr);
            if (r != DLPM_OK) return r;
        }
    }
    if (small_weight_ok(c.cout, c.cin, c.ks) && boundary == 0) {
        DLPM_HIP(hipMalloc(&c.w_rs, (size_t)small_weight_floats(c.cout, c.cin, c.ks) * sizeof(float)));
        int r = relayout_weight_small(src, c.w_rs, c.cout, c.cin, c.ks, nullptr);
        if (r != DLPM_OK) return r;
    }
    return relayout_weight(src, c.w_dev, c.cout, c.cin, c.ks, c.use_igemm, nullptr);
}

void attach_conv(const dlpm_unet *u, const ConvW &c, ConvLaunch &L) {
    policy_of(u, L);
    L.w = c.w_dev;
    L.w_frag = c.w_frag;
    L.w_wino = c.w_wino;
    L.w_wino4 = c.w_wino4;
    L.w_wino4_n64 = c.w_wino4_n64;
    L.w_wino4_n32 = c.w_wino4_n32;
    L.w_small = c.w_small;
    L.w_taps = c.w_taps;
    L.w_hfused = c.w_hfused;
    L.w_split = c.w_split;
    L.ks = c.ks;
    L.Cout = c.cout;
}

int run_conv(const dlpm_unet *u, const ConvW &c, ConvLaunch L, hipStream_t st, const HeadUpdate *hu = nullptr, float *head_scratch = nullptr) {
    policy_of(u, L);
    L.w = c.w_dev;
    L.w_frag = c.w_frag;
    L.w_wino = c.w_wino;
    L.w_wino4 = c.w_wino4;
    L.w_wino4_n64 = c.w_wino4_n64;
    L.w_wino4_n32 = c.w_wino4_n32;
    L.w_small = c.w_small;
    L.w_taps = c.w_taps;
    L.w_hfused = c.w_hfused;
    L.w_split = c.w_split;
    L.ks = c.ks;
    L.Cout = c.cout;
    if (head_fused_ok(L)) return launch_conv_head_fused(L, hu, st);
    if (head_scratch && head_gemm_ok(L)) return launch_conv_head_gemm(L, hu, head_scratch, st);
    if (head_conv_ok(L)) return launch_conv_head(L, hu, st);
    if (hu) { set_error("unet: the head convolution of this net cannot carry the fused update"); return DLPM_ERR_UNSUPPORTED; }
    return c.use_igemm ? launch_conv_igemm(L, st) : launch_conv_fallback(L, st);
}

#define TRY(expr)                  \
    do {                           \
        int _r = (expr);           \
        if (_r != DLPM_OK) return _r; \
    } while (0)

struct Ctx {
    dlpm_unet *u;
    int B;
    Bump ws;
    hipStream_t st;
    float *embout = nullptr;
    bool uniform_t = false;
    const int64_t *y = nullptr;
    int64_t emb_pitch() const { return (uniform_t && !y) ? 0 : u->emb_total; }
    const HeadUpdate *hu = nullptr;
    bool dry() const { return ws.dry; }
};

int ksplit_of(const Ctx &cx, const ConvW &c, ConvLaunch L) {
    attach_conv(cx.u, c, L);
    L.bias = nullptr;
    return conv_ksplit_for(L);
}
int run_conv3(Ctx &cx, const ConvW &c, const ConvLaunch &L) {
    const int S = ksplit_of(cx, c, L);
    if (S <= 1) return run_conv(cx.u, c, L, cx.st);
    const int64_t npix = (int64_t)L.B * L.Hout * L.Wout;
    float *part = cx.ws.alloc((int64_t)S * npix * c.cout);
    ConvLaunch P = L;
    P.bias = nullptr; P.res0 = nullptr; P.res1 = nullptr; P.R0 = 0; P.stats_out = nullptr; P.out = part; P.ksplit = S;
    int rc = run_conv(cx.u, c, P, cx.st);
    if (rc == DLPM_OK) rc = launch_splitk_reduce(part, S, npix, c.cout, L.bias, L.res0, L.res1, L.R0, L.out, cx.st);
    cx.ws.release(part);
    return rc;
}
void reserve_ksplit(Ctx &cx, const ConvW &c, const ConvLaunch &L) {
    const int S = ksplit_of(cx, c, L);
    if (S > 1) cx.ws.release(cx.ws.alloc((int64_t)S * L.B * L.Hout * L.Wout * c.cout));
}

void release_res_temps(Ctx &cx, float *cA1, float *cB1, Tensor4 &h1, float *cA2, float *cB2, float *sk) {
    cx.ws.release(cA1);
    cx.ws.release(cB1);
    drop(cx.ws, h1);
    cx.ws.release(cA2);
    cx.ws.release(cB2);
    cx.ws.release(sk);
}

int run_res(Ctx &cx, const Layer &L, Tensor4 x0, Tensor4 x1, Tensor4 *out) {
    dlpm_unet *u = cx.u;
    const int B = cx.B, H = x0.H, W = x0.W, HW = H * W;
    const int C0 = x0.C, C1 = x1.C, Cin = C0 + C1, Co = L.cout;
    {
        ResSmallLaunch r;
        r.x0 = x0.p; r.x1 = x1.p; r.C0 = C0; r.C1 = C1; r.B = B; r.H = H; r.W = W;
        r.w1f = L.c1.w_rs; r.w2f = L.c2.w_rs; r.wsf = L.has_skip ? L.skip.w_rs : nullptr;
        if (u->gen == DLPM_CONV_AUTO && Co == 64 && (!L.has_skip || r.wsf) && res_small_ok(r)) {
            float *o = cx.ws.alloc((int64_t)B * HW * Co);
            out->p = o; out->C = Co; out->H = H; out->W = W;
            out->stats = reinterpret_cast<float2 *>(cx.ws.alloc((int64_t)2 * B * Co));
            out->stats_px = HW;
            if (cx.dry()) return DLPM_OK;
            r.gn1_w = u->params[L.p_gn1_w].dev; r.gn1_b = u->params[L.p_gn1_b].dev;
            r.gn2_w = u->params[L.p_gn2_w].dev; r.gn2_b = u->params[L.p_gn2_b].dev;
            r.b1 = u->params[L.c1.p_b].dev; r.b2 = u->params[L.c2.p_b].dev;
            r.bs = L.has_skip ? u->params[L.skip.p_b].dev : nullptr;
            r.emb = cx.embout; r.emb_stride = cx.emb_pitch(); r.emb_off = L.emb_off;
            r.out = o; r.stats_out = out->stats;
// ... 314 lines not shown
                case L_STEM: convf(L.c1, H, H); break;
                case L_RES:
                    convf(L.c1, H, H); convf(L.c2, H, H);
                    if (L.has_skip) convf(L.skip, H, H);
                    break;
                case L_ATTN:
                    convf(L.c1, H, H); convf(L.c2, H, H);
                    f += 4LL * (H * H) * (H * H) * L.cin;
                    break;
                case L_DOWN: H = (H - 1) / 2 + 1; convf(L.c1, H, H); break;
                case L_UP: H *= 2; convf(L.c1, H, H); break;
            }
        }
    };
    for (auto &s : u->in_blocks) seqf(s);
    seqf(u->mid);
    for (auto &s : u->out_blocks) seqf(s);
    convf(u->head, H, H);
    return f;
}

}

static int create_net(const dlpm_unet_config *cfg, int32_t num_classes, dlpm_unet **out) {
    DLPM_CHECK_ARG(cfg && out, "dlpm_unet_create: null argument");
    DLPM_CHECK_ARG(cfg->in_channels > 0 && cfg->model_channels > 0 && cfg->out_channels > 0 && cfg->num_res_blocks > 0,
                   "dlpm_unet_create: channels / res blocks must be positive");
    DLPM_CHECK_ARG(cfg->n_mult > 0 && cfg->n_mult <= 8 && cfg->n_attn >= 0 && cfg->n_attn <= 8,
                   "dlpm_unet_create: bad channel_mult / attention_resolutions length");
    DLPM_CHECK_ARG(cfg->num_heads > 0 && cfg->image_size > 0, "dlpm_unet_create: bad num_heads / image_size");
    DLPM_CHECK_ARG(cfg->image_size % (1 << (cfg->n_mult - 1)) == 0,
                   "dlpm_unet_create: image_size %d not divisible by 2^%d (the reference UNet fails on such sizes too)",
                   cfg->image_size, cfg->n_mult - 1);
    dlpm_unet *u = new dlpm_unet();
    u->cfg = *cfg;
    u->num_classes = num_classes;
    build_arch(u);
    *out = u;
    return DLPM_OK;
}

extern "C" int dlpm_unet_create(const dlpm_unet_config *cfg, dlpm_unet **out) { return create_net(cfg, 0, out); }

extern "C" int dlpm_unet_create_conditional(const dlpm_unet_config *cfg, int32_t num_classes, dlpm_unet **out) {
    DLPM_CHECK_ARG(num_classes > 0, "dlpm_unet_create_conditional: num_classes must be positive, got %d", num_classes);
    return create_net(cfg, num_classes, out);
}

extern "C" int32_t dlpm_unet_num_classes(const dlpm_unet *net) { return net ? net->num_classes : 0; }

extern "C" int dlpm_unet_num_params(const dlpm_unet *net) { return net ? (int)net->params.size() : 0; }

extern "C" const char *dlpm_unet_param_key(const dlpm_unet *net, int i, int64_t *numel_out) {
    if (!net || i < 0 || i >= (int)net->params.size()) return nullptr;
    if (numel_out) *numel_out = net->params[i].numel;
    return net->params[i].key.c_str();
}

extern "C" int dlpm_unet_set_param(dlpm_unet *net, const char *key, const float *host, int64_t numel) {
    DLPM_CHECK_ARG(net && key && host, "dlpm_unet_set_param: null argument");
    auto it = net->index.find(key);
    DLPM_CHECK_ARG(it != net->index.end(), "dlpm_unet_set_param: unexpected key '%s' for this architecture", key);
    Param &p = net->params[it->second];
    DLPM_CHECK_ARG(p.numel == numel, "dlpm_unet_set_param: '%s' has %lld elements, expected %lld", key, (long long)numel,
                   (long long)p.numel);
    if (!p.dev) DLPM_HIP(hipMalloc(&p.dev, (size_t)numel * sizeof(float)));
    DLPM_HIP(hipMemcpy(p.dev, host, (size_t)numel * sizeof(float), hipMemcpyHostToDevice));
    p.set = true;
    net->finalized = false;
    return DLPM_OK;
}

static void free_conv(ConvW &c) {
    if (c.owns && c.w_dev) (void)hipFree(c.w_dev);
    if (c.w_frag) (void)hipFree(c.w_frag);
    c.w_frag = nullptr;
    if (c.w_wino) (void)hipFree(c.w_wino);
    c.w_wino = nullptr;
    if (c.w_wino4) (void)hipFree(c.w_wino4);
    c.w_wino4 = nullptr;
    if (c.w_wino4_n64) (void)hipFree(c.w_wino4_n64);
    if (c.w_wino4_n32) (void)hipFree(c.w_wino4_n32);
    c.w_wino4_n64 = c.w_wino4_n32 = nullptr;
    if (c.w_small) (void)hipFree(c.w_small);
    c.w_small = nullptr;
    if (c.w_taps) (void)hipFree(c.w_taps);
    c.w_taps = nullptr;
    if (c.w_rs) (void)hipFree(c.w_rs);
    c.w_rs = nullptr;
    if (c.w_hfused) (void)hipFree(c.w_hfused);
    c.w_hfused = nullptr;
    if (c.w_split) (void)hipFree(c.w_split);
    c.w_split = nullptr;
    c.w_dev = nullptr;
    c.owns = false;
}

static void for_each_conv(dlpm_unet *u, void (*fn)(ConvW &)) {
    auto seq = [&](std::vector<Layer> &s) {
        for (auto &L : s) {
            fn(L.c1);
            if (L.kind == L_RES || L.kind == L_ATTN) fn(L.c2);
            if (L.kind == L_RES && L.has_skip) fn(L.skip);
        }
    };
    for (auto &s : u->in_blocks) seq(s);
    seq(u->mid);
    for (auto &s : u->out_blocks) seq(s);
    fn(u->te0);
    fn(u->te2);
    fn(u->head);
}

constexpr int64_t NARROW_COPIES_MAX_BATCH = 512;
static int narrow_wino4_copies(dlpm_unet *u) {
    const bool want = u->dispatch_B > 0 && u->dispatch_B <= NARROW_COPIES_MAX_BATCH;
    int rc = DLPM_OK;
    auto one = [&](ConvW &c) {
        if (rc != DLPM_OK || !c.w_wino4 || c.cout % 128 != 0) return;
        if (!want) {
            if (c.w_wino4_n64) (void)hipFree(c.w_wino4_n64);
            if (c.w_wino4_n32) (void)hipFree(c.w_wino4_n32);
            c.w_wino4_n64 = c.w_wino4_n32 = nullptr;
            return;
        }
        for (int nq : {64, 32}) {
            float *&dst = nq == 64 ? c.w_wino4_n64 : c.w_wino4_n32;
            if (dst) continue;
            if (hipMalloc(&dst, (size_t)wino4_weight_floats(c.cout, c.cin) * sizeof(float)) != hipSuccess) { dst = nullptr; rc = DLPM_ERR_HIP; set_error("narrow_wino4_copies: hipMalloc failed"); return; }
            rc = relayout_weight_wino4(u->params[c.p_w].dev, dst, c.cout, c.cin, nullptr, nq);
            if (rc != DLPM_OK) return;
        }
    };
    auto seq = [&](std::vector<Layer> &s) {
        for (auto &L : s) {
            one(L.c1);
            if (L.kind == L_RES) one(L.c2);
        }
    };
    for (auto &s : u->in_blocks) seq(s);
    seq(u->mid);
    for (auto &s : u->out_blocks) seq(s);
    if (rc == DLPM_OK && hipDeviceSynchronize() != hipSuccess) { set_error("narrow_wino4_copies: synchronize failed"); rc = DLPM_ERR_HIP; }
    return rc;
}

extern "C" int dlpm_unet_finalize(dlpm_unet *u) {
    DLPM_CHECK_ARG(u, "dlpm_unet_finalize: null handle");
    for (auto &p : u->params)
        if (!p.set) {
            set_error("dlpm_unet_finalize: parameter '%s' was never set", p.key.c_str());
            return DLPM_ERR_STATE;
        }
    for_each_conv(u, free_conv);
    auto prep_seq = [&](std::vector<Layer> &s, int C0_first) -> int {
        for (size_t i = 0; i < s.size(); i++) {
            Layer &L = s[i];
            const bool cat = (i == 0 && L.kind == L_RES && C0_first > 0);
            const int C0 = cat ? C0_first : L.c1.cin;
            TRY(prep_conv(u, L.c1, L.kind == L_STEM ? L.c1.cin : C0, L.kind == L_STEM ? 1 : L.kind == L_DOWN ? 4 : 0));
            if (L.kind == L_RES || L.kind == L_ATTN) TRY(prep_conv(u, L.c2, L.c2.cin, 0));
            if (L.kind == L_RES && L.has_skip) TRY(prep_conv(u, L.skip, cat ? C0_first : L.skip.cin, 0));
        }
        return DLPM_OK;
    };
    for (auto &s : u->in_blocks) TRY(prep_seq(s, 0));
    TRY(prep_seq(u->mid, 0));
    {
        int ch = u->mid.back().cout;
        for (auto &s : u->out_blocks) {
            TRY(prep_seq(s, ch));
            ch = s[0].cout;
        }
    }
    TRY(prep_conv(u, u->te0, u->te0.cin, 3));
    TRY(prep_conv(u, u->te2, u->te2.cin, 3));
    TRY(prep_conv(u, u->head, u->head.cin, 2));
    if (u->embcat_w) (void)hipFree(u->embcat_w);
    if (u->embcat_b) (void)hipFree(u->embcat_b);
    DLPM_HIP(hipMalloc(&u->embcat_w, (size_t)u->emb_total * u->ted * sizeof(float)));
    DLPM_HIP(hipMalloc(&u->embcat_b, (size_t)u->emb_total * sizeof(float)));
    auto cat_seq = [&](std::vector<Layer> &s) -> int {
        for (auto &L : s)
            if (L.kind == L_RES) {
                DLPM_HIP(hipMemcpy(u->embcat_w + (size_t)L.emb_off * u->ted, u->params[L.p_emb_w].dev,
                                   (size_t)2 * L.cout * u->ted * sizeof(float), hipMemcpyDeviceToDevice));
                DLPM_HIP(hipMemcpy(u->embcat_b + L.emb_off, u->params[L.p_emb_b].dev, (size_t)2 * L.cout * sizeof(float),
                                   hipMemcpyDeviceToDevice));
            }
        return DLPM_OK;
    };
    for (auto &s : u->in_blocks) TRY(cat_seq(s));
    TRY(cat_seq(u->mid));
    for (auto &s : u->out_blocks) TRY(cat_seq(s));
    u->embcat.cout = u->emb_total; u->embcat.cin = u->ted; u->embcat.ks = 1;
    {
        ConvLaunch probe;
        probe.C0 = u->ted; probe.Cout = u->emb_total; probe.ks = 1;
        u->embcat.use_igemm = igemm_supported(probe);
        if (u->embcat.use_igemm) {
            u->embcat.w_dev = u->embcat_w;
        } else {
            DLPM_HIP(hipMalloc(&u->embcat.w_dev, (size_t)u->emb_total * u->ted * sizeof(float)));
            u->embcat.owns = true;
            TRY(relayout_weight(u->embcat_w, u->embcat.w_dev, u->emb_total, u->ted, 1, false, nullptr));
        }
    }
    TRY(narrow_wino4_copies(u));
    DLPM_HIP(hipDeviceSynchronize());
    u->flops = count_flops(u);
    u->finalized = true;
    u->plan_version++;
    return DLPM_OK;
}

extern "C" int dlpm_unet_set_conv_policy(dlpm_unet *u, int32_t generation, int64_t dispatch_batch) {
    DLPM_CHECK_ARG(u, "dlpm_unet_set_conv_policy: null handle");
    DLPM_CHECK_ARG(generation >= DLPM_CONV_AUTO && generation <= DLPM_CONV_IGEMM, "dlpm_unet_set_conv_policy: unknown generation %d",
                   generation);
    DLPM_CHECK_ARG(dispatch_batch >= 0, "dlpm_unet_set_conv_policy: negative dispatch batch");
    if (u->gen == generation && u->dispatch_B == dispatch_batch) return DLPM_OK;
    u->gen = generation;
    u->dispatch_B = dispatch_batch;
    u->plan_version++;
    if (u->finalized) TRY(narrow_wino4_copies(u));
    return DLPM_OK;
}

extern "C" int dlpm_unet_set_gemm_policy(dlpm_unet *u, int32_t mode) {
    DLPM_CHECK_ARG(u, "dlpm_unet_set_gemm_policy: null handle");
    DLPM_CHECK_ARG(mode >= DLPM_GEMM_AUTO && mode <= DLPM_GEMM_BF16X3, "dlpm_unet_set_gemm_policy: unknown mode %d", mode);
    if (u->gemm == mode) return DLPM_OK;
    u->gemm = mode;
    u->plan_version++;
    return DLPM_OK;
}

extern "C" int64_t dlpm_unet_time_embedding_width(const dlpm_unet *u) { return u ? u->emb_total : -1; }
extern "C" int64_t dlpm_unet_time_embeddings_scratch_bytes(const dlpm_unet *u, int64_t M) {
    return (u && M > 0) ? M * (u->cfg.model_channels + 2 * (int64_t)u->ted) * (int64_t)sizeof(float) : -1;
}

extern "C" int dlpm_unet_time_embeddings(dlpm_unet *net, const float *t_dev, int64_t M, float *out_dev, void *scratch_dev, int64_t scratch_bytes,
// ... 126 lines not shown
    }
    HeadUpdate hu;
    hu.x = upd->x_dev; hu.z = upd->z_dev; hu.t = upd->t_dev; hu.g = upd->g_dev; hu.c_eps = upd->c_eps_dev; hu.c_noise = upd->c_noise_dev;
    hu.key = upd->key_dev; hu.seed = upd->seed; hu.sample_offset = upd->sample_offset; hu.hist_pp = upd->hist_pp;
    hu.T = upd->T; hu.B = B;
    float dummy;
    int r = unet_forward(net, x_in_dev, t_dev, eps_scratch_dev ? eps_scratch_dev : &dummy, B, workspace_dev, workspace_bytes, stream, true,
                         y_dev, &hu);
    if (r != DLPM_OK) return r;
    if (upd->flags & DLPM_UPD_ADVANCE) return launch_step_advance(const_cast<int32_t *>(upd->t_dev), stream);
    return DLPM_OK;
}

static int unet_forward(dlpm_unet *net, const float *x_dev, const float *t_dev, float *eps_dev, int64_t B, void *workspace_dev,
                        int64_t workspace_bytes, dlpm_stream_t stream, bool uniform_t, const int64_t *y_dev, const HeadUpdate *hu) {
    DLPM_CHECK_ARG(net && x_dev && t_dev && eps_dev && workspace_dev, "dlpm_unet_forward: null argument");
    DLPM_CHECK_ARG(net->num_classes == 0 || y_dev, "dlpm_unet_forward: must specify y if and only if the model is class-conditional "
                   "(this net has %d classes: call the *_labels forward)", net->num_classes);
    DLPM_CHECK_ARG(net->num_classes > 0 || !y_dev, "dlpm_unet_forward: must specify y if and only if the model is class-conditional "
                   "(labels given to an unconditional net)");
    DLPM_CHECK_ARG(B > 0 && B < (1 << 24), "dlpm_unet_forward: bad batch %lld", (long long)B);
    if (!net->finalized) {
        set_error("dlpm_unet_forward: call dlpm_unet_finalize first");
        return DLPM_ERR_STATE;
    }
    const int64_t need = dlpm_unet_workspace_bytes(net, B);
    if (need < 0) return DLPM_ERR_ARG;
    if (workspace_bytes < need) {
        set_error("dlpm_unet_forward: workspace of %lld bytes, need %lld", (long long)workspace_bytes, (long long)need);
        return DLPM_ERR_NOMEM;
    }
    Ctx cx;
    cx.u = net;
    cx.B = (int)B;
    cx.ws.base = static_cast<char *>(workspace_dev);
    cx.ws.cap = workspace_bytes;
    cx.ws.reuse = !net->keep_feats;
    cx.st = as_stream(stream);
    cx.uniform_t = uniform_t;
    cx.y = y_dev;
    cx.hu = hu;
    return walk(net, cx, x_dev, t_dev, eps_dev);
}

extern "C" int dlpm_unet_keep_features(dlpm_unet *net, int on) {
    DLPM_CHECK_ARG(net, "dlpm_unet_keep_features: null handle");
    net->keep_feats = on != 0;
    net->plan_version++;
    return DLPM_OK;
}

extern "C" int dlpm_unet_num_features(const dlpm_unet *net) {
    return net ? (int)(net->in_blocks.size() + 1 + net->out_blocks.size()) : 0;
}

extern "C" int dlpm_unet_feature_shape(const dlpm_unet *net, int i, int32_t *C, int32_t *H, int32_t *W) {
    DLPM_CHECK_ARG(net && i >= 0 && i < (int)net->feats.size(), "dlpm_unet_feature_shape: no such feature (run a forward first)");
    if (C) *C = net->feats[i].C;
    if (H) *H = net->feats[i].H;
    if (W) *W = net->feats[i].W;
    return DLPM_OK;
}

extern "C" int dlpm_unet_get_feature(dlpm_unet *net, int i, float *out_nchw_dev, int64_t B, dlpm_stream_t stream) {
    DLPM_CHECK_ARG(net && out_nchw_dev && i >= 0 && i < (int)net->feats.size() && net->feats[i].p,
                   "dlpm_unet_get_feature: no such feature (call dlpm_unet_keep_features(net, 1), then run a forward)");
    const Tensor4 &f = net->feats[i];
    return dlpm_nhwc_to_nchw_f32(f.p, out_nchw_dev, (int32_t)B, f.C, f.H, f.W, stream);
}

extern "C" int64_t dlpm_unet_flops_per_sample(const dlpm_unet *net) { return net ? net->flops : 0; }

extern "C" void dlpm_unet_destroy(dlpm_unet *u) {
    if (!u) return;
    for_each_conv(u, free_conv);
    if (u->embcat.owns && u->embcat.w_dev) (void)hipFree(u->embcat.w_dev);
    if (u->embcat_w) (void)hipFree(u->embcat_w);
    if (u->embcat_b) (void)hipFree(u->embcat_b);
    for (auto &p : u->params)
        if (p.dev) (void)hipFree(p.dev);
    delete u;
}

extern "C" int dlpm_conv2d_f32(const dlpm_conv_args *a, float *scratch_dev, dlpm_stream_t stream) {
    DLPM_CHECK_ARG(a && a->src0 && a->weight && a->out && scratch_dev, "dlpm_conv2d_f32: null argument");
    DLPM_CHECK_ARG(a->ksize == 1 || a->ksize == 3, "dlpm_conv2d_f32: ksize must be 1 or 3");
    DLPM_CHECK_ARG(a->stride == 1 || a->stride == 2, "dlpm_conv2d_f32: stride must be 1 or 2");
    DLPM_CHECK_ARG((a->C1 == 0) == (a->src1 == nullptr), "dlpm_conv2d_f32: src1/C1 mismatch");
    ConvLaunch L;
    L.src0 = a->src0; L.src1 = a->src1; L.C0 = a->C0; L.C1 = a->C1; L.B = a->B;
    L.Hin = a->Hin; L.Win = a->Win; L.Hout = a->Hout; L.Wout = a->Wout;
    L.ks = a->ksize; L.stride = a->stride; L.ups = a->upsample;
    L.bias = a->bias; L.coefA = a->coefA; L.coefB = a->coefB; L.act_silu = a->act_silu;
    L.res0 = a->res0; L.res1 = a->res1; L.R0 = a->R0; L.out = a->out; L.Cout = a->Cout;
    L.in_nchw = a->in_nchw; L.out_nchw = a->out_nchw;
    const bool ig = !(a->force_direct & 1) && igemm_supported(L);
    if ((a->in_nchw || a->out_nchw) && a->C1 != 0) {
        set_error("dlpm_conv2d_f32: NCHW boundary layouts do not combine with a concat input");
        return DLPM_ERR_UNSUPPORTED;
    }
    if (a->force_direct & 4) {
        set_error("dlpm_conv2d_f32: force_direct bit 2 (value 4) asked for 1x1 convolutions on the weight-streaming kernel, which was removed");
        return DLPM_ERR_UNSUPPORTED;
    }
    hipStream_t st = as_stream(stream);
    TRY(relayout_weight(a->weight, scratch_dev, a->Cout, a->C0 + a->C1, a->ksize, ig, st));
    L.w = scratch_dev;
    L.gemm = DLPM_GEMM_F32;
    const int taps = a->ksize * a->ksize;
    if (ig && (a->force_direct & 16) && a->Cout % 128 == 0 && (a->C0 + a->C1) % 32 == 0 &&
        a->scratch_floats >= (int64_t)a->Cout * (a->C0 + a->C1) * taps + split_weight_floats(a->Cout, a->C0 + a->C1, taps)) {
        float *wsp = scratch_dev + (int64_t)a->Cout * (a->C0 + a->C1) * taps;
        TRY(relayout_weight_split(a->weight, wsp, a->Cout, a->C0 + a->C1, taps, st));
        L.w_split = wsp;
        L.gemm = DLPM_GEMM_BF16X3;
    }
    if (ig && a->ksize == 3 && !L.w_split && (a->C0 + a->C1) % 32 == 0 &&
        a->scratch_floats >= (int64_t)a->Cout * (a->C0 + a->C1) * 9 + frag_weight_floats(a->Cout, a->C0 + a->C1)) {
        float *wf = scratch_dev + (int64_t)a->Cout * (a->C0 + a->C1) * 9;
        TRY(relayout_weight_frag(a->weight, wf, a->Cout, a->C0 + a->C1, st));
        L.w_frag = wf;
        int64_t used = (int64_t)a->Cout * (a->C0 + a->C1) * 9 + frag_weight_floats(a->Cout, a->C0 + a->C1);
        const bool wino_shape = !(a->force_direct & 2) && a->stride == 1 && !a->in_nchw && !a->out_nchw;
        if (wino_shape && a->Cout % 64 == 0 && a->scratch_floats >= used + wino_weight_floats(a->Cout, a->C0 + a->C1)) {
            float *ww = scratch_dev + used;
            TRY(relayout_weight_wino(a->weight, ww, a->Cout, a->C0 + a->C1, st));
            L.w_wino = ww;
            used += wino_weight_floats(a->Cout, a->C0 + a->C1);
        }
        if (wino_shape && (a->force_direct & 8) && a->Cout % 32 == 0 && (a->C0 + a->C1) % 8 == 0 &&
            a->scratch_floats >= used + wino4_weight_floats(a->Cout, a->C0 + a->C1)) {
            float *w4 = scratch_dev + used;
            TRY(relayout_weight_wino4(a->weight, w4, a->Cout, a->C0 + a->C1, st));
            L.w_wino4 = w4;
            int bh_, bw_, ni_;
            if (!wino4_geometry(L, &bh_, &bw_, &ni_)) {
                set_error("dlpm_conv2d_f32: force_direct bit 8 asks for the F(4x4,3x3) kernel, which does not take this geometry");
                return DLPM_ERR_UNSUPPORTED;
            }
            L.w_wino = nullptr;
        }
    }
    if ((a->force_direct & 64) && a->ksize == 3 && a->Cout <= 3 && a->C0 % 32 == 0 && a->C1 == 0) {
        L.w_hfused = scratch_dev;
        L.gemm = (a->force_direct & 128) ? DLPM_GEMM_F32 : DLPM_GEMM_AUTO;
        if (a->scratch_floats >= head_fused_weight_floats(a->C0) && head_fused_ok(L)) {
            TRY(relayout_weight_head_fused(a->weight, scratch_dev, a->Cout, a->C0, st));
            return launch_conv_head_fused(L, nullptr, st);
        }
        set_error("dlpm_conv2d_f32: the one-pass head kernel does not take this shape / scratch size");
        return DLPM_ERR_UNSUPPORTED;
    }
    if ((a->force_direct & 32) && a->ksize == 3 && a->Cout <= 3 && a->C0 % 32 == 0 && a->C1 == 0) {
        const int64_t wsz = (int64_t)head_taps_rows(a->Cout) * a->C0;
        L.w_taps = scratch_dev;
        if (a->scratch_floats >= wsz + head_gemm_scratch_floats(L) && head_gemm_ok(L)) {
            TRY(relayout_weight_head_taps(a->weight, scratch_dev, a->Cout, a->C0, st));
            return launch_conv_head_gemm(L, nullptr, scratch_dev + wsz, st);
        }
        set_error("dlpm_conv2d_f32: the GEMM + gather head does not take this shape / scratch size");
        return DLPM_ERR_UNSUPPORTED;
    }
    if (!(a->force_direct & 7) && a->ksize == 3 && a->Cout <= 4 && a->C0 % 32 == 0 && a->C1 == 0) {
        const int64_t front = (int64_t)a->Cout * a->C0 * 9 + frag_weight_floats(a->Cout, a->C0);
        const int64_t wsz = (int64_t)9 * a->C0 * 4;
        if (a->scratch_floats >= front + wsz) {
            float *ws = scratch_dev + (a->scratch_floats - wsz);
            TRY(relayout_weight_head(a->weight, ws, a->Cout, a->C0, st));
            L.w_small = ws;
            if (head_conv_ok(L)) return launch_conv_head(L, nullptr, st);
        }
    }
    if (ig) return launch_conv_igemm(L, st);
    return (a->force_direct & 1) ? launch_conv_direct(L, st) : launch_conv_fallback(L, st);
}

extern "C" int dlpm_groupnorm_coeffs_f32(const float *src0, const float *src1, int32_t C0, int32_t C1, int32_t B, int32_t HW,
                                         int32_t groups, const float *gamma, const float *beta, const float *ss,
                                         int64_t ss_stride, int64_t ss_offset, float *coefA, float *coefB,
                                         dlpm_stream_t stream) {
    DLPM_CHECK_ARG(src0 && gamma && beta && coefA && coefB, "dlpm_groupnorm_coeffs_f32: null argument");
    DLPM_CHECK_ARG(groups > 0 && (C0 + C1) % groups == 0, "dlpm_groupnorm_coeffs_f32: %d channels not divisible by %d groups",
                   C0 + C1, groups);
    return launch_gn_coeffs(src0, src1, C0, C1, B, HW, groups, gamma, beta, ss, ss_stride, ss_offset, coefA, coefB,
                            as_stream(stream));
}

extern "C" int dlpm_attention_f32(const float *qkv, float *out, int32_t B, int32_t T, int32_t C, int32_t heads,
                                  dlpm_stream_t stream) {
    DLPM_CHECK_ARG(qkv && out && B > 0, "dlpm_attention_f32: null argument");
    return launch_attention(qkv, out, B, T, C, heads, as_stream(stream));
}

extern "C" int dlpm_attention_general_f32(const float *qkv, float *out, int32_t B, int32_t T, int32_t C, int32_t heads,
                                          dlpm_stream_t stream) {
    DLPM_CHECK_ARG(qkv && out && B > 0, "dlpm_attention_general_f32: null argument");
    return launch_attention_general(qkv, out, B, T, C, heads, as_stream(stream));
}

extern "C" int dlpm_resblock_small_f32(const dlpm_resblock_args *a, float *scratch_dev, int64_t scratch_floats, dlpm_stream_t stream) {
    DLPM_CHECK_ARG(a && a->x0 && a->conv1_w && a->conv2_w && a->ss && a->out && scratch_dev, "dlpm_resblock_small_f32: null argument");
    DLPM_CHECK_ARG(a->gn1_w && a->gn1_b && a->gn2_w && a->gn2_b && a->conv1_b && a->conv2_b, "dlpm_resblock_small_f32: null GroupNorm / bias parameter");
    DLPM_CHECK_ARG(!a->skip_w || a->skip_b, "dlpm_resblock_small_f32: skip_w without skip_b");
    DLPM_CHECK_ARG(a->B > 0 && a->H == a->W && (a->H == 8 || a->H == 4), "dlpm_resblock_small_f32: B %d, %d x %d images (8x8 or 4x4)", a->B, a->H, a->W);
    DLPM_CHECK_ARG((a->C1 == 0) == (a->x1 == nullptr), "dlpm_resblock_small_f32: x1/C1 mismatch");
    const int Cin = a->C0 + a->C1;
    const int64_t n1 = (int64_t)64 * Cin * 9, n2 = (int64_t)64 * 64 * 9, ns = a->skip_w ? (int64_t)64 * Cin : 0;
    DLPM_CHECK_ARG(scratch_floats >= n1 + n2 + ns, "dlpm_resblock_small_f32: scratch of %lld floats, need %lld", (long long)scratch_floats,
                   (long long)(n1 + n2 + ns));
    DLPM_CHECK_ARG(small_weight_ok(64, Cin, 3), "dlpm_resblock_small_f32: %d input channels (64 or 128)", Cin);
    hipStream_t st = as_stream(stream);
    TRY(relayout_weight_small(a->conv1_w, scratch_dev, 64, Cin, 3, st));
    TRY(relayout_weight_small(a->conv2_w, scratch_dev + n1, 64, 64, 3, st));
    if (a->skip_w) TRY(relayout_weight_small(a->skip_w, scratch_dev + n1 + n2, 64, Cin, 1, st));
    ResSmallLaunch r;
    r.x0 = a->x0; r.x1 = a->x1; r.C0 = a->C0; r.C1 = a->C1; r.B = a->B; r.H = a->H; r.W = a->W;
    r.gn1_w = a->gn1_w; r.gn1_b = a->gn1_b; r.gn2_w = a->gn2_w; r.gn2_b = a->gn2_b;
    r.w1f = scratch_dev; r.b1 = a->conv1_b; r.w2f = scratch_dev + n1; r.b2 = a->conv2_b;
    r.wsf = a->skip_w ? scratch_dev + n1 + n2 : nullptr; r.bs = a->skip_b;
    r.emb = a->ss; r.emb_stride = a->ss_stride; r.emb_off = 0;
    r.out = a->out; r.stats_out = reinterpret_cast<float2 *>(a->stats_out);
    return launch_resblock_small(r, st);
}

extern "C" int64_t dlpm_resblock_img_scratch_floats(int64_t B, int32_t Cin) {
// ... 69 lines not shown
```

include/dlpm_amd.h:

```cpp
#ifndef DLPM_AMD_H
#define DLPM_AMD_H

#include <stdint.h>

#ifdef __cplusplus
extern "C" {
#endif

typedef void *dlpm_stream_t;

enum dlpm_status {
    DLPM_OK = 0,
    DLPM_ERR_ARG = -1,
    DLPM_ERR_HIP = -2,
    DLPM_ERR_UNSUPPORTED = -3,
    DLPM_ERR_STATE = -4,
    DLPM_ERR_NOMEM = -5,
    DLPM_ERR_IO = -6
};

const char *dlpm_last_error(void);
int dlpm_abi_version(void);

int dlpm_prof_enable(int on);
// ... 186 lines not shown
int dlpm_png_write_rgb8(const uint8_t *hwc_batch, int64_t B, int32_t H, int32_t W, const char *dir,
                        int64_t first_index, int32_t level, int32_t nthreads);


typedef struct dlpm_unet_config {
    int32_t in_channels, model_channels, out_channels, num_res_blocks;
    int32_t num_heads, image_size;
    int32_t n_mult, channel_mult[8];
    int32_t n_attn, attention_resolutions[8];
} dlpm_unet_config;

typedef struct dlpm_unet dlpm_unet;

int dlpm_unet_create(const dlpm_unet_config *cfg, dlpm_unet **out);
int dlpm_unet_create_conditional(const dlpm_unet_config *cfg, int32_t num_classes, dlpm_unet **out);
int32_t dlpm_unet_num_classes(const dlpm_unet *net);
int dlpm_unet_set_param(dlpm_unet *net, const char *key, const float *host_data, int64_t numel);
int dlpm_unet_num_params(const dlpm_unet *net);
const char *dlpm_unet_param_key(const dlpm_unet *net, int index, int64_t *numel_out);
int dlpm_unet_finalize(dlpm_unet *net);
int64_t dlpm_unet_workspace_bytes(const dlpm_unet *net, int64_t B);
int dlpm_unet_forward(dlpm_unet *net, const float *x_dev, const float *t_dev, float *eps_dev, int64_t B,
                      void *workspace_dev, int64_t workspace_bytes, dlpm_stream_t stream);
int64_t dlpm_unet_time_embedding_width(const dlpm_unet *net);
int64_t dlpm_unet_time_embeddings_scratch_bytes(const dlpm_unet *net, int64_t M);
int dlpm_unet_time_embeddings(dlpm_unet *net, const float *t_dev, int64_t M, float *out_dev, void *scratch_dev, int64_t scratch_bytes,
                              dlpm_stream_t stream);
int dlpm_unet_bind_time_table(dlpm_unet *net, const float *table_dev, const int32_t *row_index_dev);
int dlpm_unet_forward_uniform_t(dlpm_unet *net, const float *x_dev, const float *t_dev, float *eps_dev, int64_t B,
                                void *workspace_dev, int64_t workspace_bytes, dlpm_stream_t stream);
int dlpm_unet_forward_labels(dlpm_unet *net, const float *x_dev, const float *t_dev, const int64_t *y_dev, float *eps_dev, int64_t B,
                             void *workspace_dev, int64_t workspace_bytes, dlpm_stream_t stream);
int dlpm_unet_forward_uniform_t_labels(dlpm_unet *net, const float *x_dev, const float *t_dev, const int64_t *y_dev, float *eps_dev,
                                       int64_t B, void *workspace_dev, int64_t workspace_bytes, dlpm_stream_t stream);
int dlpm_unet_forward_update(dlpm_unet *net, const float *x_in_dev, const float *t_dev, const dlpm_update_args *upd,
                             float *eps_scratch_dev, int64_t B, void *workspace_dev, int64_t workspace_bytes,
                             dlpm_stream_t stream);
int dlpm_unet_keep_features(dlpm_unet *net, int on);
int dlpm_unet_num_features(const dlpm_unet *net);
int dlpm_unet_feature_shape(const dlpm_unet *net, int index, int32_t *C, int32_t *H, int32_t *W);
int dlpm_unet_get_feature(dlpm_unet *net, int index, float *out_nchw_dev, int64_t B, dlpm_stream_t stream);
int64_t dlpm_unet_flops_per_sample(const dlpm_unet *net);

enum dlpm_conv_generation { DLPM_CONV_AUTO = 0, DLPM_CONV_F4 = 1, DLPM_CONV_F2 = 2, DLPM_CONV_IGEMM = 3 };
int dlpm_unet_set_conv_policy(dlpm_unet *net, int32_t generation, int64_t dispatch_batch);
enum dlpm_gemm_mode { DLPM_GEMM_AUTO = 0, DLPM_GEMM_F32 = 1, DLPM_GEMM_BF16X3 = 2 };
int dlpm_unet_set_gemm_policy(dlpm_unet *net, int32_t mode);
int64_t dlpm_unet_plan_version(const dlpm_unet *net);
void dlpm_unet_destroy(dlpm_unet *net);

typedef struct dlpm_mlp dlpm_mlp;
int dlpm_mlp_create(int32_t nfeatures, int32_t nunits, int32_t nblocks, int32_t time_emb_size, dlpm_mlp **out);
int dlpm_mlp_set_param(dlpm_mlp *net, const char *key, const float *host_data, int64_t numel);
int dlpm_mlp_finalize(dlpm_mlp *net);
int dlpm_mlp_forward(dlpm_mlp *net, const float *x_dev, const float *t_dev, float *eps_dev, int64_t B,
                     dlpm_stream_t stream);
int dlpm_mlp_sample_steps_f32(dlpm_mlp *net, float *x_dev, const float *c_eps_dev, const float *c_noise_dev,
                              const float *g_dev, int32_t T, int64_t B, int32_t t_start, int32_t nsteps,
                              uint64_t seed, int64_t sample_offset, const uint64_t *key_dev, dlpm_stream_t stream);
void dlpm_mlp_destroy(dlpm_mlp *net);


typedef struct dlpm_conv_args {
    const float *src0, *src1;
    int32_t C0, C1;
    int32_t B, Hin, Win, Hout, Wout;
    int32_t ksize;
    int32_t stride;
    int32_t upsample;
    const float *weight;
    const float *bias;
    const float *coefA, *coefB;
    int32_t act_silu;
    const float *res0, *res1;
    int32_t R0;
    float *out;
    int32_t Cout;
    int32_t in_nchw, out_nchw;
    int32_t force_direct;
    int64_t scratch_floats;
} dlpm_conv_args;

int dlpm_conv2d_f32(const dlpm_conv_args *args, float *scratch_dev, dlpm_stream_t stream);

int dlpm_groupnorm_coeffs_f32(const float *src0, const float *src1, int32_t C0, int32_t C1, int32_t B, int32_t HW,
                              int32_t groups, const float *gamma_dev, const float *beta_dev,
                              const float *ss_dev, int64_t ss_stride, int64_t ss_offset,
                              float *coefA_dev, float *coefB_dev, dlpm_stream_t stream);

int dlpm_attention_f32(const float *qkv_dev, float *out_dev, int32_t B, int32_t T, int32_t C, int32_t heads,
                       dlpm_stream_t stream);

int dlpm_attention_general_f32(const float *qkv_dev, float *out_dev, int32_t B, int32_t T, int32_t C, int32_t heads,
                               dlpm_stream_t stream);

typedef struct dlpm_resblock_args {
    const float *x0, *x1;
    int32_t C0, C1, B, H, W;
    const float *gn1_w, *gn1_b;
    const float *conv1_w, *conv1_b;
    const float *ss;
    int64_t ss_stride;
    const float *gn2_w, *gn2_b;
    const float *conv2_w, *conv2_b;
    const float *skip_w, *skip_b;
    float *out;
    float *stats_out;
} dlpm_resblock_args;
int dlpm_resblock_small_f32(const dlpm_resblock_args *args, float *scratch_dev, int64_t scratch_floats, dlpm_stream_t stream);

int64_t dlpm_resblock_img_scratch_floats(int64_t B, int32_t Cin);
int dlpm_resblock_img_f32(const dlpm_resblock_args *args, float *scratch_dev, int64_t scratch_floats, dlpm_stream_t stream);

typedef struct dlpm_attnblock_args {
    const float *x;
    int32_t C, heads, B, H, W;
    const float *gn_w, *gn_b;
    const float *qkv_w, *qkv_b;
    const float *proj_w, *proj_b;
    float *out;
    float *stats_out;
} dlpm_attnblock_args;
int dlpm_attnblock_small_f32(const dlpm_attnblock_args *args, float *scratch_dev, int64_t scratch_floats, dlpm_stream_t stream);

int dlpm_timestep_embedding_f32(const float *t_dev, float *emb_dev, int64_t B, int32_t dim, dlpm_stream_t stream);

int dlpm_nchw_to_nhwc_f32(const float *src, float *dst, int32_t B, int32_t C, int32_t H, int32_t W, dlpm_stream_t stream);
int dlpm_nhwc_to_nchw_f32(const float *src, float *dst, int32_t B, int32_t C, int32_t H, int32_t W, dlpm_stream_t stream);


typedef struct dlpm_sampler_config {
    dlpm_unet *unet;
    dlpm_mlp *mlp;
    int64_t B;
    int32_t C, H, W;
    int32_t T;
    double alpha;
    double clamp_a, clamp_eps;
    int32_t flags;
    float dlim_eta;
    uint64_t seed;
    int64_t sample_offset;
    int32_t use_graph;
    const float *g, *bg, *s, *bs;
    const float *lim_ts, *lim_tmp, *lim_cx, *lim_cs, *lim_cn;
    const float *in_scale;
    int32_t mean_type;
} dlpm_sampler_config;

typedef struct dlpm_sampler dlpm_sampler;

int dlpm_sampler_create(const dlpm_sampler_config *cfg, dlpm_sampler **out);
int dlpm_sampler_reseed(dlpm_sampler *s, uint64_t seed, int64_t sample_offset);
int dlpm_sampler_begin(dlpm_sampler *s, dlpm_stream_t stream);
int dlpm_sampler_begin_injected(dlpm_sampler *s, const float *A_dev, const float *xT_dev, dlpm_stream_t stream);
int dlpm_sampler_set_state(dlpm_sampler *s, const float *x_dev, int32_t t, dlpm_stream_t stream);
int dlpm_sampler_step_injected(dlpm_sampler *s, const float *z_dev, dlpm_stream_t stream);
int dlpm_sampler_steps(dlpm_sampler *s, int32_t nsteps, dlpm_stream_t stream);
int dlpm_sampler_set_history(dlpm_sampler *s, float *hist_dev, dlpm_stream_t stream);
int dlpm_sampler_set_labels(dlpm_sampler *s, const int64_t *y_dev, dlpm_stream_t stream);

int dlpm_sampler_copy_state(dlpm_sampler *s, float *out_dev, dlpm_stream_t stream);
float *dlpm_sampler_state(dlpm_sampler *s);
int32_t dlpm_sampler_t(const dlpm_sampler *s);
float *dlpm_sampler_table(dlpm_sampler *s, int which);
void dlpm_sampler_destroy(dlpm_sampler *s);
// ... 6 lines not shown
```

Before: 27.91.

## Add sub-pixel Winograd F(4x4) kernel for nearest-upsample 3x3 convolutions

Adds a kernel for 3x3 convolutions that follow a 2x nearest upsample. It splits the output into four sub-pixel phase classes and runs Winograd F(4x4,3x3) on the low-resolution input using per-class pre-folded weights. This avoids materialising or convolving the upsampled tensor and cuts the redundant MACs on repeated pixels. The cost is an extra per-layer weight relayout buffer and a specialised, complex kernel whose geometry checks gate when it is used.

```diff
diff --git a/dlpm_amd/_lib.py b/dlpm_amd/_lib.py
--- a/dlpm_amd/_lib.py
+++ b/dlpm_amd/_lib.py
@@ -143,6 +143,7 @@
     'dlpm_mlp_sample_steps_f32': (C.c_int, [vp, vp, vp, vp, vp, i32, i64, i32, i32, u64, i64, vp, vp]),
     'dlpm_mlp_destroy': (None, [vp]),
     'dlpm_conv2d_f32': (C.c_int, [C.POINTER(ConvArgs), vp, vp]),
+    'dlpm_conv2d_stats_f32': (C.c_int, [C.POINTER(ConvArgs), vp, vp, C.POINTER(i32), vp]),
     'dlpm_groupnorm_coeffs_f32': (C.c_int, [vp, vp, i32, i32, i32, i32, i32, vp, vp, vp, i64, i64, vp, vp, vp]),
     'dlpm_attention_f32': (C.c_int, [vp, vp, i32, i32, i32, i32, vp]),
     'dlpm_attention_general_f32': (C.c_int, [vp, vp, i32, i32, i32, i32, vp]),
diff --git a/dlpm_amd/csrc/conv.h b/dlpm_amd/csrc/conv.h
--- a/dlpm_amd/csrc/conv.h
+++ b/dlpm_amd/csrc/conv.h
@@ -13,6 +13,7 @@
     const float *w_wino = nullptr;
     const float *w_wino4 = nullptr;
     const float *w_wino4_n64 = nullptr, *w_wino4_n32 = nullptr;
+    const float *w_wino4sp = nullptr;
     const void *w_split = nullptr;
     const float *w_small = nullptr;
     const float *w_taps = nullptr;
@@ -75,6 +76,13 @@
 int launch_conv_wino4(const ConvLaunch &c, hipStream_t st);
 int64_t wino4_weight_floats(int Cout, int Cin);
 int relayout_weight_wino4(const float *oihw_dev, float *dst_dev, int Cout, int Cin, hipStream_t st, int nq = 0);
+bool wino4sp_enabled();
+bool wino4sp_layer_ok(int Cout, int Cin, int Hlo, int Wlo);
+bool wino4sp_geometry(const ConvLaunch &c, int *bh, int *bw, int *nimg);
+bool wino4sp_preferred(const ConvLaunch &c, int *bh, int *bw, int *nimg);
+int launch_conv_wino4sp(const ConvLaunch &c, hipStream_t st);
+int64_t wino4sp_weight_floats(int Cout, int Cin);
+int relayout_weight_wino4sp(const float *oihw_dev, float *dst_dev, int Cout, int Cin, hipStream_t st);
 struct ResImgLaunch {
     const float *x0 = nullptr, *x1 = nullptr;
     int C0 = 0, C1 = 0, B = 0;
diff --git a/dlpm_amd/csrc/conv_igemm.hip b/dlpm_amd/csrc/conv_igemm.hip
--- a/dlpm_amd/csrc/conv_igemm.hip
+++ b/dlpm_amd/csrc/conv_igemm.hip
@@ -1019,6 +1019,7 @@
         const int64_t hw = (int64_t)c.Hout * c.Wout;
         return (c.R0 & 3) ? 0 : hw % BM == 0 ? BM : hw == 64 ? 64 : 0;
     }
+    if (wino4sp_preferred(c, &a, &b, &n)) return n == 1 ? 256 : (n == 4 && a * b == 4) ? 64 : 0;
     if (wino4_preferred(c, &a, &b, &n)) return n == 1 ? 256 : (n == 4 && a * b == 4) ? 64 : 0;
     if (wino_geometry(c, &a, &b, &n)) return n == 1 ? 4 * wino_tiles(c) : 0;
     if (c.out_nchw || (c.Cout & 3) || (c.R0 & 3)) return 0;
@@ -1051,6 +1052,14 @@
     }
     {
         int wb, ww, wi;
+        if (wino4sp_preferred(c, &wb, &ww, &wi)) {
+            if (prof_enabled() && prof_detail())
+                snprintf(pname, sizeof(pname), "conv3x3_wino4sp:H%d:Cin%d+%d:Cout%d:u%d:coef%d", c.Hout, c.C0, c.C1, c.Cout, c.ups, c.coefA ? 1 : 0);
+            else
+                snprintf(pname, sizeof(pname), "conv3x3_wino4sp");
+            ProfScope psw(pname, 2.0 * M * c.Cout * K, bytes, st);
+            return launch_conv_wino4sp(c, st);
+        }
         if (wino4_preferred(c, &wb, &ww, &wi)) {
             if (prof_enabled() && prof_detail())
                 snprintf(pname, sizeof(pname), "conv3x3_wino4:H%d:Cin%d+%d:Cout%d:u%d:coef%d", c.Hout, c.C0, c.C1, c.Cout, c.ups, c.coefA ? 1 : 0);
diff --git a/dlpm_amd/csrc/conv_wino4.hip b/dlpm_amd/csrc/conv_wino4.hip
--- a/dlpm_amd/csrc/conv_wino4.hip
+++ b/dlpm_amd/csrc/conv_wino4.hip
@@ -206,6 +206,44 @@
 __device__ __forceinline__ int f4_item_src(int iv) { return (iv >> 14) & 1023; }
 __device__ __forceinline__ bool f4_item_pad(int iv) { return iv & (1 << 24); }
 __device__ __forceinline__ bool f4_item_none(int iv) { return iv & (1 << 25); }
+
+__device__ __forceinline__ void fs_v_row_out(const float2 (&T)[5], int ra, float *vb, int vpp) {
+    const float2 e1 = f4_bt_part<1>(T[2], T[4]), o1 = f4_bt_part<1>(T[1], T[3]);
+    const float2 e2 = f4_bt_part<3>(T[2], T[4]), o2 = f4_bt_part<3>(T[1], T[3]);
+    const float2 v[5] = {f4_bt_end(T[0], T[2], T[4]), f4_bt_plus<1>(o1, e1), f4_bt_minus<1>(o1, e1), f4_bt_plus<3>(o2, e2), f4_bt_minus<3>(o2, e2)};
+#pragma unroll
+    for (int rb = 0; rb < 5; rb++) {
+        const int pos = 5 * ra + rb;
+        *reinterpret_cast<float2 *>(vb + (pos >> 1) * vpp + (pos & 1) * 2) = v[rb];
+    }
+}
+template <class D>
+__device__ __forceinline__ void fs_transform_rp(int rp, const D &d, float *vb, int vpp) {
+    float2 Ta[5], Tb[5];
+    if (rp == 0) {
+#pragma unroll
+        for (int c = 0; c < 5; c++) Ta[c] = f4_bt_outer<0>(d, c);
+        fs_v_row_out(Ta, 0, vb, vpp);
+    } else if (rp == 1) {
+#pragma unroll
+        for (int c = 0; c < 5; c++) f4_bt_mid<1>(d, c, Ta[c], Tb[c]);
+        fs_v_row_out(Ta, 1, vb, vpp);
+        fs_v_row_out(Tb, 2, vb, vpp);
+    } else {
+#pragma unroll
+        for (int c = 0; c < 5; c++) f4_bt_mid<3>(d, c, Ta[c], Tb[c]);
+        fs_v_row_out(Ta, 3, vb, vpp);
+        fs_v_row_out(Tb, 4, vb, vpp);
+    }
+}
+__device__ __forceinline__ void fs_out_tile(const floatx4 (&acc)[25], int r, float (&Yt)[16]) {
+    float Z[4][5];
+#pragma unroll
+    for (int b = 0; b < 5; b++)
+        f4_at(acc[0 * 5 + b][r], acc[1 * 5 + b][r], acc[2 * 5 + b][r], acc[3 * 5 + b][r], acc[4 * 5 + b][r], 0.f, Z[0][b], Z[1][b], Z[2][b], Z[3][b]);
+#pragma unroll
+    for (int i = 0; i < 4; i++) f4_at(Z[i][0], Z[i][1], Z[i][2], Z[i][3], Z[i][4], 0.f, Yt[i * 4 + 0], Yt[i * 4 + 1], Yt[i * 4 + 2], Yt[i * 4 + 3]);
+}
 
 template <bool UPS, int QN = F4_QNIT, int NW = 8>
 __global__ void __launch_bounds__((NW + (NW == 8 ? 0 : NW == 4 ? 3 : 2)) * 64, NW == 2 ? 2 : 1) k_conv3x3_wino4(ConvLaunch p_in, int bh_in, int bw_in, int nimg_in) {
@@ -506,6 +544,264 @@
 #ifdef DLPM_PHASE_DEFER
     if (p.phase && lane == 0) atomicAdd(p.phase + 16 + wave, (unsigned long long)_wait);
 #endif
+#ifdef DLPM_PHASE_TIMING
+    if (p.phase && tid == 0) {
+        atomicAdd(p.phase + 11, 1ull);
+        atomicAdd(p.phase + 12, (unsigned long long)(clock64() - _c0));
+        atomicAdd(p.phase + 13, (unsigned long long)(wall_clock64() - _r0));
+    }
+#endif
+}
+
+constexpr int FS_PP = 12;
+constexpr int FS_FRAGS = 13;
+constexpr int FS_VPP = 4 * F4_TILES * 4;
+constexpr int FS_VBUF = FS_FRAGS * FS_VPP;
+constexpr int FS_RAWPIX = 352;
+constexpr int FS_RAWBUF = FS_RAWPIX * F4_PRLD + 16;
+constexpr int FS_PAD = 16;
+constexpr int FS_S0 = 4, FS_X = 9;
+static_assert(FS_PP % F4_RING == 0, "a fragment's ring slot must not depend on the phase");
+
+__global__ void __launch_bounds__(F4_NT, 1) k_conv3x3_wino4sp(ConvLaunch p_in, int bh_in, int bw_in, int nimg_in) {
+    constexpr int QN = 2;
+    ConvLaunch p = p_in;
+    const int bh = bh_in, bw = bw_in, nimg = nimg_in;
+    extern __shared__ __attribute__((aligned(16))) float wsm[];
+    float *V = wsm;
+    float *raw = wsm + 2 * FS_VBUF;
+    float *Cf = raw + 2 * FS_RAWBUF;
+
+    DLPM_PHASE_DECL;
+#ifdef DLPM_PHASE_TIMING
+    const long long _c0 = clock64(), _r0 = wall_clock64();
+#endif
+    const int tid = threadIdx.x, lane = tid & 63, wave = tid >> 6;
+    const int li = lane & 15, lk = lane >> 4;
+    const int W = p.Wout, H = p.Hout, Ws = p.Win, Hs = p.Hin, TW = Ws >> 2, TH = Hs >> 2;
+    const int Cin = p.C0 + p.C1;
+    const int nch = Cin / F4_KC;
+    const unsigned bid = blockIdx.x;
+    const int ntn = p.Cout / F4_NQ;
+    const int nmb = (gridDim.x >> 2) / ntn;
+    const int cls = bid & 3, mb = (bid >> 2) % nmb, nt = (bid >> 2) / nmb;
+    const int ca = cls >> 1, cb = cls & 1, n0 = nt * F4_NQ;
+    int img0, ty0, tx0, blk_in_img = 0;
+    const int bpr = TW / bw, bpi = (TH / bh) * bpr;
+    if (nimg == 1) {
+        img0 = mb / bpi;
+        blk_in_img = mb - img0 * bpi;
+        ty0 = (blk_in_img / bpr) * bh;
+        tx0 = (blk_in_img % bpr) * bw;
+    } else {
+        img0 = mb * nimg;
+        ty0 = tx0 = 0;
+    }
+    const int RH = 4 * bh + 1, RW = 4 * bw + 1;
+    const int oy = 4 * ty0 - 1 + ca, ox = 4 * tx0 - 1 + cb;
+    const int rpi = RH * RW, npix = nimg * rpi;
+
+    const int squad = tid & 1;
+    auto pix_of = [&](int it) { return it == 1 ? (F4_NT / 2) + ((F4_NT - 1 - tid) >> 1) : (tid >> 1); };
+    const bool skewed = nimg == 1 && bh <= 4;
+    int off[QN], lo[QN];
+#pragma unroll
+    for (int it = 0; it < QN; it++) {
+        const int pix = pix_of(it);
+        const int img = min(pix / rpi, nimg - 1), r = pix - img * rpi;
+        const int ry = r / RW, rx = r - ry * RW;
+        const int iy = oy + ry, ix = ox + rx;
+        const bool pad = iy < 0 || iy >= Hs || ix < 0 || ix >= Ws || (img0 + img) >= p.B;
+        off[it] = pix >= npix ? -2 : (pad ? -1 : (((img0 + img) * Hs + iy) * Ws + ix));
+        lo[it] = (pix * F4_PRLD + squad * 4 + (skewed ? 4 * (ry >> 2) : 0)) | ((img * 2 * F4_KC + squad * 4) << 16);
+    }
+    const bool has_coef = p.coefA != nullptr;
+    const int cf_img = tid >> 2, cf_isb = (tid >> 1) & 1;
+    const bool cf_mine = has_coef && tid < nimg * 4;
+    const float *cf_base = has_coef ? ((cf_isb ? p.coefB : p.coefA) + (int64_t)min(img0 + cf_img, p.B - 1) * Cin + squad * 4) : nullptr;
+    float4 xr[QN], cfr = make_float4(0.f, 0.f, 0.f, 0.f);
+    auto load_raw_into = [&](float4 (&dst)[QN], int chunk) {
+        const int c = chunk * F4_KC + squad * 4;
+        const bool first = c < p.C0;
+        const float *sb = first ? p.src0 + c : p.src1 + (c - p.C0);
+        const int ld = first ? p.C0 : p.C1;
+#pragma unroll
+        for (int it = 0; it < QN; it++) dst[it] = *reinterpret_cast<const float4 *>(sb + (int64_t)max(off[it], 0) * ld);
+    };
+    auto load_coef = [&](int chunk) {
+        if (cf_mine) cfr = *reinterpret_cast<const float4 *>(cf_base + chunk * F4_KC);
+    };
+    auto store_coef = [&](int slot) {
+        if (cf_mine) *reinterpret_cast<float4 *>(Cf + slot * F4_CFS + cf_img * 2 * F4_KC + cf_isb * F4_KC + squad * 4) = cfr;
+    };
+    auto store_raw_item = [&](int slot, int it) {
+        if (off[it] == -2) return;
+        float *rb = raw + slot * FS_RAWBUF;
+        float4 x = xr[it];
+        if (has_coef) {
+            const float4 ca4 = *reinterpret_cast<const float4 *>(Cf + slot * F4_CFS + (lo[it] >> 16));
+            const float4 cb4 = *reinterpret_cast<const float4 *>(Cf + slot * F4_CFS + (lo[it] >> 16) + F4_KC);
+            x = f4_affine4(x, ca4, cb4);
+        }
+        if (p.act_silu) x = f4_silu4(x);
+        if (off[it] < 0) x = make_float4(0.f, 0.f, 0.f, 0.f);
+        *reinterpret_cast<float4 *>(rb + (lo[it] & 0xffff)) = x;
+    };
+    auto store_raw = [&](int slot) {
+#pragma unroll
+        for (int it = 0; it < QN; it++) store_raw_item(slot, it);
+    };
+
+    int rbase, vofs;
+    {
+        const int tile = lane & 15, pair = lane >> 4;
+        const int timg = tile / (bh * bw), r = tile - timg * (bh * bw);
+        const int ty = r / bw, tx = r - ty * bw;
+        rbase = (timg * rpi + 4 * ty * RW + 4 * tx) * F4_PRLD + pair * 2 + (skewed ? 4 * ty : 0);
+        vofs = (pair * F4_TILES + tile) * 4;
+    }
+    auto transform = [&](int slot) {
+        if (wave < 3) fs_transform_rp(wave, F4Patch<false, F4_PRLD>{raw + slot * FS_RAWBUF + rbase, RW, skewed}, V + slot * FS_VBUF + vofs, FS_VPP);
+    };
+
+    const float4 *__restrict__ wp = reinterpret_cast<const float4 *>(p.w_wino4sp) +
+                                    ((int64_t)((cls * ntn + nt) * 8 + __builtin_amdgcn_readfirstlane(wave)) * nch) * FS_FRAGS * 64;
+    constexpr int AHEAD = F4_RING - 1;
+    float4 bq[F4_RING];
+    float2 bt;
+    const float *asrc = V + lane * 4;
+
+    floatx4 acc[25];
+#pragma unroll
+    for (int q = 0; q < 25; q++)
+#pragma unroll
+        for (int r = 0; r < 4; r++) acc[q][r] = 0.f;
+
+    const int last = nch - 1;
+    float4 xr1[QN], cfr1 = make_float4(0.f, 0.f, 0.f, 0.f), cfr2 = cfr1;
+    load_raw_into(xr, 0);
+    load_raw_into(xr1, min(1, last));
+    load_coef(0);
+    if (cf_mine) {
+        cfr1 = *reinterpret_cast<const float4 *>(cf_base + min(1, last) * F4_KC);
+        cfr2 = *reinterpret_cast<const float4 *>(cf_base + min(2, last) * F4_KC);
+    }
+#pragma unroll
+    for (int a = 0; a < AHEAD; a++) bq[a] = wp[a * 64 + lane];
+    bt = *reinterpret_cast<const float2 *>(wp + FS_PP * 64 + lane);
+    store_coef(0);
+    cfr = cfr1;
+    store_coef(1);
+    __syncthreads();
+    store_raw(0);
+#pragma unroll
+    for (int it = 0; it < QN; it++) xr[it] = xr1[it];
+    store_raw(1);
+    load_raw_into(xr, min(2, last));
+    __syncthreads();
+    transform(0);
+    cfr = cfr2;
+    store_coef(0);
+    __syncthreads();
+    DLPM_PHASE(p, 8);
+
+#pragma unroll 1
+    for (int chunk = 0; chunk < nch; chunk++) {
+        const int cur = chunk & 1, nxt = cur ^ 1;
+        const float *ab = asrc + cur * FS_VBUF;
+        load_coef(min(chunk + 3, last));
+        float4 aq[2];
+        float2 at;
+        aq[0] = *reinterpret_cast<const float4 *>(ab);
+        const float2 btn = *reinterpret_cast<const float2 *>(wp + (FS_FRAGS + FS_PP) * 64 + lane);
+#pragma unroll
+        for (int pp = 0; pp < FS_PP; pp++) {
+            if (pp >= FS_S0 && pp < FS_S0 + QN) store_raw_item(cur, pp - FS_S0);
+            if (pp == FS_S0 + QN) load_raw_into(xr, min(chunk + 3, last));
+            if (pp == FS_X) transform(nxt);
+            {
+                const int f = pp + AHEAD;
+                bq[f % F4_RING] = wp[(f < FS_PP ? f : f + 1) * 64 + lane];
+            }
+            if (pp + 1 < FS_PP) aq[(pp + 1) & 1] = *reinterpret_cast<const float4 *>(ab + (pp + 1) * FS_VPP);
+            else at = *reinterpret_cast<const float2 *>(ab + FS_PP * FS_VPP);
+            if (F4_PRIO) __builtin_amdgcn_s_setprio(0);
+            f4_mfma4(aq[pp & 1], bq[pp % F4_RING], acc[2 * pp], acc[2 * pp + 1]);
+            if (pp == FS_PP - 1) {
+                acc[24] = __builtin_amdgcn_mfma_f32_16x16x4f32(at.x, bt.x, acc[24], 0, 0, 0);
+                acc[24] = __builtin_amdgcn_mfma_f32_16x16x4f32(at.y, bt.y, acc[24], 0, 0, 0);
+            }
+            if (F4_PRIO) __builtin_amdgcn_s_setprio(1);
+        }
+        bt = btn;
+        wp += FS_FRAGS * 64;
+        store_coef(nxt);
+        __syncthreads();
+    }
+    if (F4_PRIO) __builtin_amdgcn_s_setprio(0);
+    DLPM_PHASE(p, 9);
+
+    const int64_t pix0 = ((int64_t)img0 * H + 8 * ty0 + ca) * W + 8 * tx0 + cb;
+    const int ch = n0 + 16 * wave + li;
+    const float bias_v = p.bias ? p.bias[ch] : 0.f;
+    const bool has_res = p.res0 != nullptr;
+    const bool res_first = __builtin_amdgcn_readfirstlane(n0 + 16 * wave) < p.R0;
+    const float *res_u = has_res ? (res_first ? p.res0 : p.res1 - p.R0) : nullptr;
+    const int res_ld = res_first ? p.R0 : p.Cout - p.R0;
+    const int lbw = 31 - __builtin_clz(bw), lbhw = 31 - __builtin_clz(bh * bw);
+    float *__restrict__ out_blk = p.out + pix0 * p.Cout;
+    const float *__restrict__ res_blk = has_res ? res_u + pix0 * res_ld : nullptr;
+    const bool img_stats = p.stats_out != nullptr && nimg == 4 && bh * bw == 4;
+    const bool do_stats = (p.stats_out != nullptr && nimg == 1) || img_stats;
+    float K = 0.f, s1 = 0.f, s2 = 0.f;
+#pragma unroll
+    for (int r = 0; r < 4; r++) {
+        const int tile = 4 * lk + r;
+        const int timg = tile >> lbhw, ty = (tile & (bh * bw - 1)) >> lbw, tx = tile & (bw - 1);
+        const int tpix = (timg * H + 8 * ty) * W + 8 * tx;
+        const bool ok = img0 + timg < p.B;
+        float rs[16];
+        const uint32_t bo_o = (uint32_t)(tpix * p.Cout + ch) * 4u, bo_r = (uint32_t)(tpix * res_ld + ch) * 4u;
+        if (has_res && ok) {
+#pragma unroll
+            for (int i = 0; i < 4; i++)
+#pragma unroll
+                for (int j = 0; j < 4; j++)
+                    rs[i * 4 + j] = *reinterpret_cast<const float *>(reinterpret_cast<const char *>(res_blk + (2 * i * W + 2 * j) * res_ld) + bo_r);
+        }
+        float Yt[16];
+        fs_out_tile(acc, r, Yt);
+        if (!ok) continue;
+#pragma unroll
+        for (int i = 0; i < 4; i++) {
+            const float *y = Yt + 4 * i;
+#pragma unroll
+            for (int j = 0; j < 4; j++) {
+                float v = y[j] + bias_v;
+                if (has_res) v += rs[i * 4 + j];
+                if (do_stats) {
+                    if (r == 0 && i == 0 && j == 0) K = v;
+                    const float dd = v - K;
+                    s1 += dd;
+                    s2 = fmaf(dd, dd, s2);
+                }
+                *reinterpret_cast<float *>(reinterpret_cast<char *>(out_blk + (2 * i * W + 2 * j) * p.Cout) + bo_o) = v;
+            }
+        }
+    }
+    if (img_stats) {
+        if (img0 + lk < p.B) {
+            float mean, M2;
+            f4_stats_lane<64>(K, s1, s2, mean, M2);
+            p.stats_out[((int64_t)(img0 + lk) * 4 + cls) * p.Cout + ch] = make_float2(mean, M2);
+        }
+    } else if (do_stats) {
+        float mean, M2;
+        f4_stats_merge<64>(K, s1, s2, lane, mean, M2);
+        if (lk == 0) p.stats_out[(((int64_t)img0 * bpi + blk_in_img) * 4 + cls) * p.Cout + ch] = make_float2(mean, M2);
+    }
+    DLPM_PHASE(p, 10);
+    DLPM_PHASE_FLUSH(p, 8);
 #ifdef DLPM_PHASE_TIMING
     if (p.phase && tid == 0) {
         atomicAdd(p.phase + 11, 1ull);
@@ -1157,6 +1453,38 @@
     dst[i] = (float)u;
 }
 
+__global__ void k_relayout_weight_wino4sp(const float *oihw, float *dst, int Cout, int Cin) {
+    const int nch = Cin / F4_KC;
+    const int64_t total = (int64_t)4 * Cout * Cin * 26;
+    const int64_t i = (int64_t)blockIdx.x * blockDim.x + threadIdx.x;
+    if (i >= total) return;
+    const int e = (int)(i & 3);
+    const int lane = (int)((i >> 2) & 63);
+    int64_t r = i >> 8;
+    const int pp = (int)(r % FS_FRAGS); r /= FS_FRAGS;
+    const int chunk = (int)(r % nch); r /= nch;
+    const int wave = (int)(r % 8); r /= 8;
+    const int ntn = Cout / F4_NQ;
+    const int nt = (int)(r % ntn);
+    const int cls = (int)(r / ntn), ca = cls >> 1, cb = cls & 1;
+    const int lk = lane >> 4, li = lane & 15;
+    const int pos = 2 * pp + (e >> 1);
+    if (pos >= 25) { dst[i] = 0.f; return; }
+    const int cin = chunk * F4_KC + 2 * lk + (e & 1);
+    const int cout = nt * F4_NQ + wave * 16 + li;
+    const float *g = oihw + ((int64_t)cout * Cin + cin) * 9;
+    double ef[2][2] = {{0., 0.}, {0., 0.}};
+    for (int ii = 0; ii < 3; ii++)
+        for (int jj = 0; jj < 3; jj++) ef[ca ? (ii == 2) : (ii != 0)][cb ? (jj == 2) : (jj != 0)] += (double)g[ii * 3 + jj];
+    const double a = F4_PA, b = F4_PB, a2 = a * a, b2 = b * b;
+    const double n0 = a2 * b2, na = 2. * a2 * (a2 - b2), nb = 2. * b2 * (b2 - a2);
+    const double G[5][2] = {{1. / n0, 0.}, {1. / na, a / na}, {1. / na, -a / na}, {1. / nb, b / nb}, {1. / nb, -b / nb}};
+    const int ra = pos / 5, rb = pos % 5;
+    double u = 0.;
+    for (int ii = 0; ii < 2; ii++) u += G[ra][ii] * (ef[ii][0] * G[rb][0] + ef[ii][1] * G[rb][1]);
+    dst[i] = (float)u;
+}
+
 int f4_mode() {
     static int v = -1;
     if (v < 0) { const char *e = getenv("DLPM_WINO_F4"); v = e ? atoi(e) : 1; }
@@ -1354,4 +1682,75 @@
     return DLPM_OK;
 }
 
-}
+bool wino4sp_enabled() {
+    static int v = -1;
+    if (v < 0) { const char *e = getenv("DLPM_WINO4_SUBPIX"); v = e ? atoi(e) : 1; }
+    return v != 0 && wino4_enabled();
+}
+
+static bool wino4sp_block(int Cout, int Cin, int Hlo, int Wlo, int *bh, int *bw, int *nimg) {
+    if (Cout % F4_NQ != 0 || Cin % F4_KC != 0 || Hlo <= 0 || Wlo <= 0 || (Hlo & 3) || (Wlo & 3)) return false;
+    const int TH = Hlo / 4, TW = Wlo / 4;
+    int h, w, n;
+    if (TH * TW >= F4_TILES) {
+        w = TW < 4 ? TW : 4;
+        if (F4_TILES % w != 0) return false;
+        h = F4_TILES / w;
+        if (TW % w != 0 || TH % h != 0) return false;
+        n = 1;
+    } else {
+        if (F4_TILES % (TH * TW) != 0) return false;
+        h = TH; w = TW; n = F4_TILES / (TH * TW);
+    }
+    if (n > 4) return false;
+    if (n * (4 * h + 1) * (4 * w + 1) > FS_RAWPIX) return false;
+    *bh = h; *bw = w; *nimg = n;
+    return true;
+}
+bool wino4sp_layer_ok(int Cout, int Cin, int Hlo, int Wlo) {
+    int h, w, n;
+    return wino4sp_enabled() && wino4sp_block(Cout, Cin, Hlo, Wlo, &h, &w, &n);
+}
+
+bool wino4sp_geometry(const ConvLaunch &c, int *bh, int *bw, int *nimg) {
+    if (!c.ups || !c.w_wino4sp || c.ks != 3 || c.stride != 1 || c.in_nchw || c.out_nchw) return false;
+    if (c.Hout != 2 * c.Hin || c.Wout != 2 * c.Win || c.C0 % F4_KC != 0 || (c.R0 & 15) != 0 || c.ksplit > 1) return false;
+    return wino4sp_block(c.Cout, c.C0 + c.C1, c.Hin, c.Win, bh, bw, nimg);
+}
+
+bool wino4sp_preferred(const ConvLaunch &c, int *bh, int *bw, int *nimg) {
+    int a, b, n;
+    if (!c.ups || !c.w_wino4sp || !wino4sp_enabled() || !wino4_preferred(c, &a, &b, &n) || wino4_nq_for(c) != F4_NQ) return false;
+    return wino4sp_geometry(c, bh, bw, nimg);
+}
+
+int launch_conv_wino4sp(const ConvLaunch &c, hipStream_t st) {
+    int bh, bw, nimg;
+    if (!wino4sp_geometry(c, &bh, &bw, &nimg)) {
+        set_error("launch_conv_wino4sp: unsupported shape");
+        return DLPM_ERR_UNSUPPORTED;
+    }
+#ifdef DLPM_PHASE_TIMING
+    const_cast<ConvLaunch &>(c).phase = phase_buffer();
+#endif
+    const int64_t tiles = (int64_t)c.B * (c.Hin / 4) * (c.Win / 4);
+    const int64_t mblocks = nimg == 1 ? tiles / F4_TILES : ceil_div(c.B, nimg);
+    const int r = ensure_dynamic_lds(reinterpret_cast<const void *>(&k_conv3x3_wino4sp), 160 * 1024);
+    if (r != DLPM_OK) return r;
+    const size_t lds = (size_t)(2 * FS_VBUF + 2 * FS_RAWBUF + 2 * F4_CFS) * sizeof(float);
+    k_conv3x3_wino4sp<<<(unsigned)(mblocks * (c.Cout / F4_NQ) * 4), F4_NT, lds, st>>>(c, bh, bw, nimg);
+    DLPM_LAUNCH_CHECK();
+    return DLPM_OK;
+}
+
+int64_t wino4sp_weight_floats(int Cout, int Cin) { return (int64_t)4 * Cout * Cin * 26 + FS_PAD * 256; }
+
+int relayout_weight_wino4sp(const float *oihw_dev, float *dst_dev, int Cout, int Cin, hipStream_t st) {
+    const int64_t n = (int64_t)4 * Cout * Cin * 26;
+    DLPM_HIP(hipMemsetAsync(dst_dev + n, 0, (size_t)FS_PAD * 256 * sizeof(float), st));
+    k_relayout_weight_wino4sp<<<(unsigned)ceil_div(n, 256), 256, 0, st>>>(oihw_dev, dst_dev, Cout, Cin);
+    DLPM_LAUNCH_CHECK();
+    return DLPM_OK;
+}
+
+}
diff --git a/dlpm_amd/csrc/unet.hip b/dlpm_amd/csrc/unet.hip
--- a/dlpm_amd/csrc/unet.hip
+++ b/dlpm_amd/csrc/unet.hip
@@ -29,6 +29,7 @@
     float *w_wino = nullptr;
     float *w_wino4 = nullptr;
     float *w_wino4_n64 = nullptr, *w_wino4_n32 = nullptr;
+    float *w_wino4sp = nullptr;
     float *w_small = nullptr;
     float *w_taps = nullptr;
     void *w_split = nullptr;
@@ -109,7 +110,7 @@
     t.stats_px = 0;
     if (off || (!c.use_igemm && !stem)) return;
     ConvLaunch L;
-    L.w_wino = c.w_wino; L.w_wino4 = c.w_wino4; L.w_wino4_n64 = c.w_wino4_n64; L.w_wino4_n32 = c.w_wino4_n32; L.w_split = c.w_split; L.ks = c.ks; L.stride = stride; L.ups = ups; L.Hout = t.H; L.Wout = t.W; L.Cout = c.cout;
+    L.w_wino = c.w_wino; L.w_wino4 = c.w_wino4; L.w_wino4_n64 = c.w_wino4_n64; L.w_wino4_n32 = c.w_wino4_n32; L.w_wino4sp = c.w_wino4sp; L.w_split = c.w_split; L.ks = c.ks; L.stride = stride; L.ups = ups; L.Hout = t.H; L.Wout = t.W; L.Cout = c.cout;
     L.Hin = ups ? t.H / 2 : t.H * stride; L.Win = ups ? t.W / 2 : t.W * stride;
     L.C0 = C0; L.C1 = c.cin - C0; L.B = B;
     L.in_nchw = stem ? 1 : 0;
@@ -285,7 +286,7 @@
     u->head = u->conv("out.2.", c.out_channels, mc, 3);
 }
 
-int prep_conv(dlpm_unet *u, ConvW &c, int C0, int boundary) {
+int prep_conv(dlpm_unet *u, ConvW &c, int C0, int boundary, int ups_lo = 0) {
     ConvLaunch probe;
     probe.C0 = C0; probe.C1 = c.cin - C0; probe.Cout = c.cout; probe.ks = c.ks;
     probe.in_nchw = boundary == 1; probe.out_nchw = boundary == 2;
@@ -339,6 +340,11 @@
             DLPM_HIP(hipMalloc(&c.w_wino4, (size_t)wino4_weight_floats(c.cout, c.cin) * sizeof(float)));
             r = relayout_weight_wino4(src, c.w_wino4, c.cout, c.cin, nullptr);
             if (r != DLPM_OK) return r;
+            if (ups_lo > 0 && wino4sp_layer_ok(c.cout, c.cin, ups_lo, ups_lo)) {
+                DLPM_HIP(hipMalloc(&c.w_wino4sp, (size_t)wino4sp_weight_floats(c.cout, c.cin) * sizeof(float)));
+                r = relayout_weight_wino4sp(src, c.w_wino4sp, c.cout, c.cin, nullptr);
+                if (r != DLPM_OK) return r;
+            }
         }
     }
     if (small_weight_ok(c.cout, c.cin, c.ks) && boundary == 0) {
@@ -357,6 +363,7 @@
     L.w_wino4 = c.w_wino4;
     L.w_wino4_n64 = c.w_wino4_n64;
     L.w_wino4_n32 = c.w_wino4_n32;
+    L.w_wino4sp = c.w_wino4sp;
     L.w_small = c.w_small;
     L.w_taps = c.w_taps;
     L.w_hfused = c.w_hfused;
@@ -373,6 +380,7 @@
     L.w_wino4 = c.w_wino4;
     L.w_wino4_n64 = c.w_wino4_n64;
     L.w_wino4_n32 = c.w_wino4_n32;
+    L.w_wino4sp = c.w_wino4sp;
     L.w_small = c.w_small;
     L.w_taps = c.w_taps;
     L.w_hfused = c.w_hfused;
@@ -853,6 +861,8 @@
     if (c.w_wino4_n64) (void)hipFree(c.w_wino4_n64);
     if (c.w_wino4_n32) (void)hipFree(c.w_wino4_n32);
     c.w_wino4_n64 = c.w_wino4_n32 = nullptr;
+    if (c.w_wino4sp) (void)hipFree(c.w_wino4sp);
+    c.w_wino4sp = nullptr;
     if (c.w_small) (void)hipFree(c.w_small);
     c.w_small = nullptr;
     if (c.w_taps) (void)hipFree(c.w_taps);
@@ -924,12 +934,15 @@
             return DLPM_ERR_STATE;
         }
     for_each_conv(u, free_conv);
+    int res = u->cfg.image_size;
     auto prep_seq = [&](std::vector<Layer> &s, int C0_first) -> int {
         for (size_t i = 0; i < s.size(); i++) {
             Layer &L = s[i];
             const bool cat = (i == 0 && L.kind == L_RES && C0_first > 0);
             const int C0 = cat ? C0_first : L.c1.cin;
-            TRY(prep_conv(u, L.c1, L.kind == L_STEM ? L.c1.cin : C0, L.kind == L_STEM ? 1 : L.kind == L_DOWN ? 4 : 0));
+            TRY(prep_conv(u, L.c1, L.kind == L_STEM ? L.c1.cin : C0, L.kind == L_STEM ? 1 : L.kind == L_DOWN ? 4 : 0, L.kind == L_UP ? res : 0));
+            if (L.kind == L_DOWN) res = (res - 1) / 2 + 1;
+            if (L.kind == L_UP) res *= 2;
             if (L.kind == L_RES || L.kind == L_ATTN) TRY(prep_conv(u, L.c2, L.c2.cin, 0));
             if (L.kind == L_RES && L.has_skip) TRY(prep_conv(u, L.skip, cat ? C0_first : L.skip.cin, 0));
         }
@@ -1222,7 +1235,15 @@
     delete u;
 }
 
+static int conv2d_entry(const dlpm_conv_args *a, float *scratch_dev, float *stats_out, int32_t *stats_px, dlpm_stream_t stream);
 extern "C" int dlpm_conv2d_f32(const dlpm_conv_args *a, float *scratch_dev, dlpm_stream_t stream) {
+    return conv2d_entry(a, scratch_dev, nullptr, nullptr, stream);
+}
+extern "C" int dlpm_conv2d_stats_f32(const dlpm_conv_args *a, float *scratch_dev, float *stats_out, int32_t *stats_px, dlpm_stream_t stream) {
+    DLPM_CHECK_ARG(stats_out && stats_px, "dlpm_conv2d_stats_f32: null argument");
+    return conv2d_entry(a, scratch_dev, stats_out, stats_px, stream);
+}
+static int conv2d_entry(const dlpm_conv_args *a, float *scratch_dev, float *stats_out, int32_t *stats_px, dlpm_stream_t stream) {
     DLPM_CHECK_ARG(a && a->src0 && a->weight && a->out && scratch_dev, "dlpm_conv2d_f32: null argument");
     DLPM_CHECK_ARG(a->ksize == 1 || a->ksize == 3, "dlpm_conv2d_f32: ksize must be 1 or 3");
     DLPM_CHECK_ARG(a->stride == 1 || a->stride == 2, "dlpm_conv2d_f32: stride must be 1 or 2");
@@ -1255,32 +1276,57 @@
         L.w_split = wsp;
         L.gemm = DLPM_GEMM_BF16X3;
     }
-    if (ig && a->ksize == 3 && !L.w_split && (a->C0 + a->C1) % 32 == 0 &&
-        a->scratch_floats >= (int64_t)a->Cout * (a->C0 + a->C1) * 9 + frag_weight_floats(a->Cout, a->C0 + a->C1)) {
-        float *wf = scratch_dev + (int64_t)a->Cout * (a->C0 + a->C1) * 9;
-        TRY(relayout_weight_frag(a->weight, wf, a->Cout, a->C0 + a->C1, st));
+    const int Cin_ = a->C0 + a->C1;
+    int64_t used = (int64_t)a->Cout * Cin_ * taps;
+    const bool wino_shape = a->ksize == 3 && !L.w_split && !(a->force_direct & 2) && a->stride == 1 && !a->in_nchw && !a->out_nchw;
+    if (ig && a->ksize == 3 && !L.w_split && Cin_ % 32 == 0 &&
+        a->scratch_floats >= used + frag_weight_floats(a->Cout, Cin_)) {
+        float *wf = scratch_dev + used;
+        TRY(relayout_weight_frag(a->weight, wf, a->Cout, Cin_, st));
         L.w_frag = wf;
-        int64_t used = (int64_t)a->Cout * (a->C0 + a->C1) * 9 + frag_weight_floats(a->Cout, a->C0 + a->C1);
-        const bool wino_shape = !(a->force_direct & 2) && a->stride == 1 && !a->in_nchw && !a->out_nchw;
-        if (wino_shape && a->Cout % 64 == 0 && a->scratch_floats >= used + wino_weight_floats(a->Cout, a->C0 + a->C1)) {
+        used += frag_weight_floats(a->Cout, Cin_);
+        if (wino_shape && a->Cout % 64 == 0 && a->scratch_floats >= used + wino_weight_floats(a->Cout, Cin_)) {
             float *ww = scratch_dev + used;
-            TRY(relayout_weight_wino(a->weight, ww, a->Cout, a->C0 + a->C1, st));
+            TRY(relayout_weight_wino(a->weight, ww, a->Cout, Cin_, st));
             L.w_wino = ww;
-            used += wino_weight_floats(a->Cout, a->C0 + a->C1);
-        }
-        if (wino_shape && (a->force_direct & 8) && a->Cout % 32 == 0 && (a->C0 + a->C1) % 8 == 0 &&
-            a->scratch_floats >= used + wino4_weight_floats(a->Cout, a->C0 + a->C1)) {
-            float *w4 = scratch_dev + used;
-            TRY(relayout_weight_wino4(a->weight, w4, a->Cout, a->C0 + a->C1, st));
-            L.w_wino4 = w4;
-            int bh_, bw_, ni_;
-            if (!wino4_geometry(L, &bh_, &bw_, &ni_)) {
-                set_error("dlpm_conv2d_f32: force_direct bit 8 asks for the F(4x4,3x3) kernel, which does not take this geometry");
-                return DLPM_ERR_UNSUPPORTED;
-            }
-            L.w_wino = nullptr;
-        }
-    }
+            used += wino_weight_floats(a->Cout, Cin_);
+        }
+    }
+    if (wino_shape && (a->force_direct & (8 | 256)) && a->Cout % 32 == 0 && Cin_ % 8 == 0 &&
+        a->scratch_floats >= used + wino4_weight_floats(a->Cout, Cin_)) {
+        float *w4 = scratch_dev + used;
+        TRY(relayout_weight_wino4(a->weight, w4, a->Cout, Cin_, st));
+        L.w_wino4 = w4;
+        int bh_, bw_, ni_;
+        if (!wino4_geometry(L, &bh_, &bw_, &ni_)) {
+            set_error("dlpm_conv2d_f32: force_direct bit 8 asks for the F(4x4,3x3) kernel, which does not take this geometry");
+            return DLPM_ERR_UNSUPPORTED;
+        }
+        L.w_wino = nullptr;
+        used += wino4_weight_floats(a->Cout, Cin_);
+    }
+    if (a->force_direct & 256) {
+        int bh_, bw_, ni_;
+        if (L.w_wino4 && a->Cout % 128 == 0 && a->scratch_floats >= used + wino4sp_weight_floats(a->Cout, Cin_)) {
+            L.w_wino4sp = scratch_dev + used;
+            if (wino4sp_preferred(L, &bh_, &bw_, &ni_)) TRY(relayout_weight_wino4sp(a->weight, scratch_dev + used, a->Cout, Cin_, st));
+            else L.w_wino4sp = nullptr;
+        }
+        if (!L.w_wino4sp) {
+            set_error("dlpm_conv2d_f32: force_direct bit 256 asks for the sub-pixel upsampling kernel, which does not take this geometry / scratch size");
+            return DLPM_ERR_UNSUPPORTED;
+        }
+    }
+    if (stats_out) {
+        const int px = L.w_wino4 ? conv_stats_pixels(L) : 0;
+        if (px <= 0) {
+            set_error("dlpm_conv2d_stats_f32: this launch emits no statistics (Winograd F(4x4) kernels on whole blocks or whole 8x8 images only)");
+            return DLPM_ERR_UNSUPPORTED;
+        }
+        L.stats_out = reinterpret_cast<float2 *>(stats_out);
+        *stats_px = px;
+    }
+    if (L.w_wino4 && !ig) return L.w_wino4sp ? launch_conv_wino4sp(L, st) : launch_conv_wino4(L, st);
     if ((a->force_direct & 64) && a->ksize == 3 && a->Cout <= 3 && a->C0 % 32 == 0 && a->C1 == 0) {
         L.w_hfused = scratch_dev;
         L.gemm = (a->force_direct & 128) ? DLPM_GEMM_F32 : DLPM_GEMM_AUTO;
diff --git a/include/dlpm_amd.h b/include/dlpm_amd.h
--- a/include/dlpm_amd.h
+++ b/include/dlpm_amd.h
@@ -292,6 +292,7 @@
 } dlpm_conv_args;
 
 int dlpm_conv2d_f32(const dlpm_conv_args *args, float *scratch_dev, dlpm_stream_t stream);
+int dlpm_conv2d_stats_f32(const dlpm_conv_args *args, float *scratch_dev, float *stats_out, int32_t *stats_px, dlpm_stream_t stream);
 
 int dlpm_groupnorm_coeffs_f32(const float *src0, const float *src1, int32_t C0, int32_t C1, int32_t B, int32_t HW,
                               int32_t groups, const float *gamma_dev, const float *beta_dev,
```

Result: faster. 28.21, median of 6 (+1.1%).
